# diver-j/melgan-multi

Hardware: NVIDIA H100
Metric: generator_fwd_audio_frames_per_sec (higher is better)
Workload: dtype f32 in/out; products as 3 split-bf16 wgmma passes with fp32 accumulation (fp32-equivalent, ~1e-5)

## Files before the change

### include/melgan_b200.h

```cpp
#ifndef MELGAN_B200_H_
#define MELGAN_B200_H_

#include <stddef.h>
#include <stdint.h>

#ifdef __cplusplus
extern "C" {
#endif

#define MG_OK 0
#define MG_ERR_INVALID_ARGUMENT (-1)
#define MG_ERR_CUDA (-2)
#define MG_ERR_UNSUPPORTED_DEVICE (-3)
#define MG_ERR_WORKSPACE_TOO_SMALL (-4)
#define MG_ERR_OUT_OF_MEMORY (-5)

#define MG_GEN_NUM_LAYERS 30

int mg_abi_version(void);

const char *mg_last_error_string(void);

int mg_device_check(void);

size_t mg_gen_packed_bytes(void);
int mg_gen_pack(const float *const *v, const float *const *g, const float *const *bias,
                void *packed, void *stream);

size_t mg_gen_workspace_bytes(int B, int T);
int mg_gen_forward(const void *packed, const float *mel, float *audio, int B, int T,
                   void *workspace, size_t workspace_bytes, void *stream);

#define MG_GEN_RAGGED_MAX_B 256
int mg_gen_forward_ragged(const void *packed, const float *mel, float *audio, int B, int T_max, const int *lengths,
                          void *workspace, size_t workspace_bytes, void *stream);

int mg_gen_forward_timed(const void *packed, const float *mel, float *audio, int B, int T,
                         void *workspace, size_t workspace_bytes, void *stream, float *kernel_ms);

int mg_gen_check_status(const void *workspace, int B, int T, void *stream);

int mg_gen_convt(const void *packed, int stage, const float *x, float *y, int B, int Lin, void *stream);

int mg_gen_resblock(const void *packed, int stage, const float *x, float *y, int B, int L, void *stream);
int mg_gen_upres(const void *packed, int stage, const float *x, float *y, int B, int Lin, void *stream);
int mg_gen_upres_post(const void *packed, const float *x, float *audio, int B, int Lin, void *stream);
const char *mg_gen_resblock_config(int code);
const char *mg_gen_convt_config(int stage);

int mg_gen_resup(const void *packed, int stage, const float *x, float *y, int B, int L, void *stream);

int mg_gen_conv_pre(const void *packed, const float *mel, float *y, int B, int T, void *stream);
int mg_gen_resblock_post(const void *packed, const float *x, float *audio, int B, int L, void *stream);

int mg_gen_resblock_trace(const void *packed, int stage, const float *x, float *y, int B, int L, long long *trace_host);

int mg_gen_stage_output(const void *workspace, int which, float *out, int B, int T, void *stream);

size_t mg_msd_packed_bytes(void);
int mg_msd_pack(const float *const *v, const float *const *g, const float *const *bias, void *packed, void *stream);
int mg_msd_lengths(int L, int *lens);
int mg_msd_forward(const void *packed, const float *y, int Bt, int L, float *const *fmaps, void *status_word, void *stream);
int mg_msd_check_status(const void *status_word, void *stream);

size_t mg_disc_packed_bytes(void);
int mg_disc_pack(const float *const *v, const float *const *g, const float *const *bias, void *packed, void *stream);
int mg_disc_forward(const void *packed, const float *x, int Bt, int L, float *const *fmaps, void *status_word, void *stream);

size_t mg_mel_tables_bytes(void);
int mg_mel_tables_build(int sampling_rate, int n_mels, float fmin, float fmax, int norm, void *tables_host);
int mg_mel_frames(int L);
int mg_mel_spectrogram(const void *tables, const float *audio, float *mel, int B, int L, void *stream);

typedef struct mg_gen_engine mg_gen_engine;

int mg_gen_engine_create(mg_gen_engine **out, int max_B, int max_T);
int mg_gen_engine_load_state(mg_gen_engine *e, const float *const *v, const float *const *g,
                             const float *const *bias);
int mg_gen_engine_forward(mg_gen_engine *e, const float *mel_host, float *audio_host, int B, int T);
int mg_gen_engine_forward_ragged(mg_gen_engine *e, const float *mel_host, float *audio_host, int B, int T_max,
                                 const int *lengths);
int mg_gen_engine_last_kernel_ms(mg_gen_engine *e, float *ms);
void mg_gen_engine_destroy(mg_gen_engine *e);


size_t mg_msd_scale_backward_workspace_bytes(int Bt, int L0);
int mg_msd_scale_backward(const void *packed, int scale, const float *x0, const float *const *fmap, const float *const *gfmap,
                          float *gx0, float *const *dw, float *const *db, int *reached, void *workspace, size_t workspace_bytes,
                          int Bt, int L0, void *status_word, void *stream);

int mg_lrelu_backward(const float *g1, const float *g2, const float *out, float *dz, long long n, void *stream);

size_t mg_msd_grouped_backward_workspace_bytes(int layer, int Bt, int Lout);
int mg_msd_grouped_backward(const void *packed, int scale, int layer, const float *dz, const float *x, float *dx, float *dw,
                            float *db, void *workspace, size_t workspace_bytes, int Bt, int Lin, int Lout, void *stream);

int mg_msd_post1_dgrad(const void *packed, int scale, const float *dz, float *dx, int Bt, int L, void *status_word, void *stream);
int mg_msd_post1_wgrad(const float *x, const float *dz, float *dw, float *db, int Bt, int L, void *status_word, void *stream);

size_t mg_msd_edge_backward_workspace_bytes(int layer, int Bt, int L);
int mg_msd_edge_backward(const void *packed, int scale, int layer, const float *dz, const float *x, float *dx, float *dw, float *db,
                         void *workspace, size_t workspace_bytes, int Bt, int L, void *stream);

int mg_msd_wn_backward(const float *const *v, const float *const *g, const float *const *dw, float *const *dv,
                       float *const *dg, void *stream);

int mg_adam_chunk(void);
int mg_adam_step(float *const *p, const float *const *g, float *const *m, float *const *v, const long long *n,
                 const int *first, int count, int total_ctas, float lr, float beta1, float beta2, float eps,
                 float weight_decay, long long step, void *stream);

size_t mg_loss_workspace_bytes(const long long *n, int count);
int mg_loss_forward(const float *const *a, const float *const *b, const long long *n, const int *mode, int count,
                    float *out, void *workspace, size_t workspace_bytes, void *stream);
int mg_loss_backward(const float *const *a, const float *const *b, const long long *n, const int *mode, int count,
                     const float *grad_out, float *const *grad_a, float *const *grad_b, void *stream);

int mg_gen_forward_launches(void);
int mg_gen_forward_slices(int B, int T);
int mg_gen_set_pipeline(int tail_mask);
const char *mg_gen_kernel_name(int i);
const char *mg_gen_kernel_config(int i, int T);

#ifdef __cplusplus
}
#endif
#endif
```

### melgan_multi_b200/csrc/mg_api.cu

```cuda
#include <new>
#include <stdlib.h>
#include <string.h>

#include "mg_common.cuh"

namespace mg {


static int *status_ptr(void *workspace, int B, int T) {
    return reinterpret_cast<int *>(reinterpret_cast<float *>(workspace) + ws_offset(6, (size_t)B, (size_t)T));
}

static int run_generator(const float *packed, const float *mel, float *audio, const RunTable &batch, float *ws, cudaStream_t s,
                         cudaEvent_t *ev, const float *mel_host = nullptr, float *audio_host = nullptr) {
    int *st = status_ptr(ws, batch.items(), batch.stride);
    MG_CUDA_TRY(cudaMemsetAsync(st, 0, sizeof(int), s));
    return launch_generator_tc(packed, mel, audio, batch, ws, st, s, ev, mel_host, audio_host);
}

static int check_shape(const char *fn, int B, int T) {
    if (B < 1 || T < 1) return set_error(MG_ERR_INVALID_ARGUMENT, "%s: need B >= 1 and T >= 1 (got B=%d, T=%d)", fn, B, T);
    if ((long long)B * T > (1ll << 24)) return set_error(MG_ERR_INVALID_ARGUMENT, "%s: B*T = %lld too large", fn, (long long)B * T);
    return MG_OK;
}

static int check_lengths(const char *fn, int B, int T_max, const int *lengths) {
    int rc = check_shape(fn, B, T_max);
    if (rc) return rc;
    if (B > MG_GEN_RAGGED_MAX_B)
        return set_error(MG_ERR_INVALID_ARGUMENT, "%s: B = %d exceeds MG_GEN_RAGGED_MAX_B = %d", fn, B, MG_GEN_RAGGED_MAX_B);
    if (!lengths) return set_error(MG_ERR_INVALID_ARGUMENT, "%s: null lengths", fn);
    for (int i = 0; i < B; ++i)
        if (lengths[i] < 1 || lengths[i] > T_max)
            return set_error(MG_ERR_INVALID_ARGUMENT, "%s: lengths[%d] = %d is outside [1, T_max = %d]", fn, i, lengths[i], T_max);
    return MG_OK;
}

template <class F>
static int run_one_kernel(const char *fn, cudaStream_t stream, F launch) {
    int *st = nullptr;
    MG_CUDA_TRY(cudaMalloc(&st, sizeof(int)));
    cudaMemsetAsync(st, 0, sizeof(int), stream);
    int rc = launch(st);
    int h = 0;
    if (rc == MG_OK) {
        cudaError_t e = cudaStreamSynchronize(stream);
        if (e != cudaSuccess) rc = set_error(MG_ERR_CUDA, "%s: %s", fn, cudaGetErrorString(e));
        else if (cudaMemcpy(&h, st, sizeof(int), cudaMemcpyDeviceToHost) != cudaSuccess || h)
            rc = set_error(MG_ERR_CUDA, "%s: pipeline wait timed out (role code %d)", fn, h);
    }
    cudaFree(st);
    return rc;
}

}

using namespace mg;

extern "C" {

int mg_abi_version(void) { return 2; }

const char *mg_last_error_string(void) { return error_buffer(); }

int mg_device_check(void) {
    int dev = 0;
    MG_CUDA_TRY(cudaGetDevice(&dev));
    cudaDeviceProp p;
    MG_CUDA_TRY(cudaGetDeviceProperties(&p, dev));
    if (p.major != 9 || p.minor != 0)
        return set_error(MG_ERR_UNSUPPORTED_DEVICE, "device %d is sm_%d%d; this library is built for sm_90a (H100) only",
                         dev, p.major, p.minor);
    return MG_OK;
}

size_t mg_gen_packed_bytes(void) { return packed_total_bytes(); }

int mg_gen_pack(const float *const *v, const float *const *g, const float *const *bias, void *packed, void *stream) {
    if (!v || !g || !bias || !packed) return set_error(MG_ERR_INVALID_ARGUMENT, "mg_gen_pack: null argument");
    if ((uintptr_t)packed % 16) return set_error(MG_ERR_INVALID_ARGUMENT, "mg_gen_pack: packed must be 16-byte aligned");
    return launch_pack(v, g, bias, (float *)packed, (cudaStream_t)stream);
}

size_t mg_gen_workspace_bytes(int B, int T) {
    if (B < 1 || T < 1) return 0;
    return ws_offset(6, (size_t)B, (size_t)T) * sizeof(float) + 256;
}

static int check_forward(const char *fn, const void *packed, const float *mel, float *audio, int B, int T, void *workspace,
                         size_t workspace_bytes) {
    if (!packed || !mel || !audio || !workspace) return set_error(MG_ERR_INVALID_ARGUMENT, "%s: null argument", fn);
    if (workspace_bytes < mg_gen_workspace_bytes(B, T))
        return set_error(MG_ERR_WORKSPACE_TOO_SMALL, "%s: workspace %zu < %zu bytes", fn, workspace_bytes, mg_gen_workspace_bytes(B, T));
    if ((uintptr_t)packed % 16 || (uintptr_t)workspace % 16)
        return set_error(MG_ERR_INVALID_ARGUMENT, "%s: packed/workspace must be 16-byte aligned", fn);
    return MG_OK;
}

int mg_gen_forward(const void *packed, const float *mel, float *audio, int B, int T, void *workspace,
                   size_t workspace_bytes, void *stream) {
    int rc = check_shape("mg_gen_forward", B, T);
    if (!rc) rc = check_forward("mg_gen_forward", packed, mel, audio, B, T, workspace, workspace_bytes);
    if (rc) return rc;
    return run_generator((const float *)packed, mel, audio, RunTable::uniform(B, T), (float *)workspace, (cudaStream_t)stream,
                         nullptr);
}

int mg_gen_forward_ragged(const void *packed, const float *mel, float *audio, int B, int T_max, const int *lengths,
                          void *workspace, size_t workspace_bytes, void *stream) {
    int rc = check_lengths("mg_gen_forward_ragged", B, T_max, lengths);
    if (!rc) rc = check_forward("mg_gen_forward_ragged", packed, mel, audio, B, T_max, workspace, workspace_bytes);
    if (rc) return rc;
    return run_generator((const float *)packed, mel, audio, RunTable::ragged(lengths, B, T_max), (float *)workspace,
                         (cudaStream_t)stream, nullptr);
}

int mg_gen_forward_timed(const void *packed, const float *mel, float *audio, int B, int T, void *workspace,
                         size_t workspace_bytes, void *stream, float *kernel_ms) {
    int rc = check_shape("mg_gen_forward_timed", B, T);
    if (rc) return rc;
    if (!packed || !mel || !audio || !workspace || !kernel_ms)
        return set_error(MG_ERR_INVALID_ARGUMENT, "mg_gen_forward_timed: null argument");
    if (workspace_bytes < mg_gen_workspace_bytes(B, T))
        return set_error(MG_ERR_WORKSPACE_TOO_SMALL, "mg_gen_forward_timed: workspace too small");
    const int n = mg_gen_forward_launches();
    cudaEvent_t ev[17];
    for (int i = 0; i <= n; ++i) MG_CUDA_TRY(cudaEventCreate(&ev[i]));
    rc = run_generator((const float *)packed, mel, audio, RunTable::uniform(B, T), (float *)workspace, (cudaStream_t)stream, ev);
    if (rc == MG_OK) {
        cudaError_t e = cudaEventSynchronize(ev[n]);
        if (e != cudaSuccess) rc = set_error(MG_ERR_CUDA, "mg_gen_forward_timed: %s", cudaGetErrorString(e));
        for (int i = 0; i < n && rc == MG_OK; ++i)
            if (cudaEventElapsedTime(&kernel_ms[i], ev[i], ev[i + 1]) != cudaSuccess)
                rc = set_error(MG_ERR_CUDA, "mg_gen_forward_timed: cudaEventElapsedTime failed");
    }
    for (int i = 0; i <= n; ++i) cudaEventDestroy(ev[i]);
    return rc;
}

const char *mg_gen_kernel_name(int i) { return generator_tc_kernel_name(i); }

const char *mg_gen_kernel_config(int i, int T) { return generator_tc_kernel_config(i, T); }

int mg_gen_set_pipeline(int tail_mask) {
    if (tail_mask < -1 || tail_mask > 15) return set_error(MG_ERR_INVALID_ARGUMENT, "mg_gen_set_pipeline: mask %d", tail_mask);
    generator_tc_set_tail(tail_mask);
    return MG_OK;
}

int mg_gen_stage_output(const void *workspace, int which, float *out, int B, int T, void *stream) {
    int rc = check_shape("mg_gen_stage_output", B, T);
    if (rc) return rc;
    if (which < 0 || which > 3 || !workspace || !out)
        return set_error(MG_ERR_INVALID_ARGUMENT, "mg_gen_stage_output: which must be 0..3 (the last stage is fused with conv_post)");
    if (which > 0 && generator_tc_tail() != 0)
        return set_error(MG_ERR_INVALID_ARGUMENT, "mg_gen_stage_output: ResBlock outputs are not materialised while the next stage's "
                         "ConvT is fused at their kernel's tail; select the unfused chain with mg_gen_set_pipeline(0) first");
    const size_t off = ws_offset(which, B, T), n = ws_offset(which + 1, B, T) - off;
    MG_CUDA_TRY(cudaMemcpyAsync(out, (const float *)workspace + off, n * sizeof(float), cudaMemcpyDeviceToDevice,
                                (cudaStream_t)stream));
    return MG_OK;
}

size_t mg_msd_grouped_backward_workspace_bytes(int layer, int Bt, int Lout) {
    if (layer < 1 || layer > 4 || Bt < 1 || Lout < 1) return 0;
    return grouped_bwd_workspace_bytes(layer, Bt, Lout);
}

int mg_msd_grouped_backward(const void *packed, int scale, int layer, const float *dz, const float *x, float *dx, float *dw,
                            float *db, void *workspace, size_t workspace_bytes, int Bt, int Lin, int Lout, void *stream) {
    if (!packed || !dz || scale < 0 || scale > 2 || layer < 1 || layer > 4 || Bt < 1 || Lin < 1 || Lout < 1)
        return set_error(MG_ERR_INVALID_ARGUMENT, "mg_msd_grouped_backward: bad argument");
    const DLayer d = d_layer(layer);
    if (Lout != (Lin + 2 * d.pad - d.k) / d.stride + 1)
        return set_error(MG_ERR_INVALID_ARGUMENT, "mg_msd_grouped_backward: Lout %d does not follow from Lin %d", Lout, Lin);
    if (dw && (!x || !db || !workspace || workspace_bytes < grouped_bwd_workspace_bytes(layer, Bt, Lout)))
        return set_error(MG_ERR_WORKSPACE_TOO_SMALL, "mg_msd_grouped_backward: dw needs x, db and a workspace of %zu bytes",
                         grouped_bwd_workspace_bytes(layer, Bt, Lout));
    const uint8_t *blob = reinterpret_cast<const uint8_t *>(packed) + (size_t)scale * d_blob_bytes();
    return launch_disc_grouped_backward(blob, layer, dz, x, dx, dw, db, (float *)workspace, Bt, Lin, Lout, (cudaStream_t)stream);
}

int mg_msd_post1_dgrad(const void *packed, int scale, const float *dz, float *dx, int Bt, int L, void *status_word, void *stream) {
    if (!packed || !dz || !dx || dz == dx || !status_word || scale < 0 || scale > 2 || Bt < 1 || L < 1)
        return set_error(MG_ERR_INVALID_ARGUMENT, "mg_msd_post1_dgrad: bad argument");
    const uint8_t *blob = reinterpret_cast<const uint8_t *>(packed) + (size_t)scale * d_blob_bytes();
    return launch_disc_post1_dgrad_tc(dz, dx, blob + d_tcT_start(), reinterpret_cast<const float *>(blob + d_zero_start()), Bt, L,
                                      (int *)status_word, (cudaStream_t)stream);
}

int mg_msd_post1_wgrad(const float *x, const float *dz, float *dw, float *db, int Bt, int L, void *status_word, void *stream) {
    if (!x || !dz || !dw || !db || !status_word || Bt < 1 || L < 1)
        return set_error(MG_ERR_INVALID_ARGUMENT, "mg_msd_post1_wgrad: bad argument");
    return launch_disc_post1_wgrad_tc(x, dz, dw, db, Bt, L, (int *)status_word, (cudaStream_t)stream);
}

size_t mg_msd_edge_backward_workspace_bytes(int layer, int Bt, int L) {
    return (layer == 0 && Bt > 0 && L > 0) ? edge_bwd_workspace_bytes(layer, Bt, L) : 0;
}

int mg_msd_edge_backward(const void *packed, int scale, int layer, const float *dz, const float *x, float *dx, float *dw, float *db,
                         void *workspace, size_t workspace_bytes, int Bt, int L, void *stream) {
    if (!packed || !dz || !x || !dw || !db || scale < 0 || scale > 2 || (layer != 0 && layer != 6) || Bt < 1 || L < 1)
        return set_error(MG_ERR_INVALID_ARGUMENT, "mg_msd_edge_backward: bad argument (layer is 0 = conv_pre or 6 = conv_post2)");
    if (layer == 0 && (!workspace || workspace_bytes < edge_bwd_workspace_bytes(0, Bt, L)))
        return set_error(MG_ERR_WORKSPACE_TOO_SMALL, "mg_msd_edge_backward: conv_pre needs a workspace of %zu bytes",
                         edge_bwd_workspace_bytes(0, Bt, L));
    const uint8_t *blob = reinterpret_cast<const uint8_t *>(packed) + (size_t)scale * d_blob_bytes();
    return launch_disc_edge_backward(blob, layer, dz, x, dx, dw, db, (float *)workspace, Bt, L, (cudaStream_t)stream);
}

size_t mg_msd_scale_backward_workspace_bytes(int Bt, int L0) {
    return (Bt > 0 && L0 > 0) ? disc_scale_backward_workspace_bytes(Bt, L0) : 0;
}

int mg_msd_scale_backward(const void *packed, int scale, const float *x0, const float *const *fmap, const float *const *gfmap,
                          float *gx0, float *const *dw, float *const *db, int *reached, void *workspace, size_t workspace_bytes,
                          int Bt, int L0, void *status_word, void *stream) {
    if (!packed || !x0 || !fmap || !gfmap || !dw || !db || !workspace || !status_word || scale < 0 || scale > 2 || Bt < 1 || L0 < 1)
        return set_error(MG_ERR_INVALID_ARGUMENT, "mg_msd_scale_backward: bad argument");
    for (int l = 0; l < kDiscLayers; ++l)
        if (!fmap[l]) return set_error(MG_ERR_INVALID_ARGUMENT, "mg_msd_scale_backward: fmap[%d] is NULL", l);
    if (Bt > 65535) return set_error(MG_ERR_INVALID_ARGUMENT, "discriminator batch %d exceeds 65535", Bt);
    const uint8_t *blob = reinterpret_cast<const uint8_t *>(packed) + (size_t)scale * d_blob_bytes();
    return launch_disc_scale_backward(blob, x0, fmap, gfmap, gx0, dw, db, reached, workspace, workspace_bytes, Bt, L0,
                                      (int *)status_word, (cudaStream_t)stream);
}

int mg_lrelu_backward(const float *g1, const float *g2, const float *out, float *dz, long long n, void *stream) {
    return launch_lrelu_grad(g1, g2, out, dz, n, (cudaStream_t)stream);
}

int mg_msd_wn_backward(const float *const *v, const float *const *g, const float *const *dw, float *const *dv,
                       float *const *dg, void *stream) {
    if (!v || !g || !dw || !dv || !dg) return set_error(MG_ERR_INVALID_ARGUMENT, "mg_msd_wn_backward: null argument");
    return launch_disc_wn_backward(v, g, dw, dv, dg, (cudaStream_t)stream);
}

int mg_adam_chunk(void) { return 4096; }

int mg_adam_step(float *const *p, const float *const *g, float *const *m, float *const *v, const long long *n,
                 const int *first, int count, int total_ctas, float lr, float beta1, float beta2, float eps,
                 float weight_decay, long long step, void *stream) {
    return launch_adam(p, g, m, v, n, first, count, total_ctas, lr, beta1, beta2, eps, weight_decay, step, (cudaStream_t)stream);
}

size_t mg_loss_workspace_bytes(const long long *n, int count) {
    if (!n || count < 1) return 0;
    return (size_t)loss_num_ctas(n, count) * sizeof(float);
}

int mg_loss_forward(const float *const *a, const float *const *b, const long long *n, const int *mode, int count,
                    float *out, void *workspace, size_t workspace_bytes, void *stream) {
    if (!out || !workspace) return set_error(MG_ERR_INVALID_ARGUMENT, "mg_loss_forward: null argument");
    if (n && count >= 1 && workspace_bytes < mg_loss_workspace_bytes(n, count))
        return set_error(MG_ERR_WORKSPACE_TOO_SMALL, "mg_loss_forward: workspace too small");
    return launch_loss_forward(a, b, n, mode, count, out, (float *)workspace, (cudaStream_t)stream);
}

int mg_loss_backward(const float *const *a, const float *const *b, const long long *n, const int *mode, int count,
                     const float *grad_out, float *const *grad_a, float *const *grad_b, void *stream) {
    if (!grad_out) return set_error(MG_ERR_INVALID_ARGUMENT, "mg_loss_backward: null grad_out");
    return launch_loss_backward(a, b, n, mode, count, grad_out, grad_a, grad_b, (cudaStream_t)stream);
}

int mg_gen_forward_launches(void) { return generator_tc_num_launches(); }

int mg_gen_forward_slices(int B, int T) { return (B >= 1 && T >= 1) ? generator_tc_slices(B, (long long)B * T) : 1; }

int mg_gen_check_status(const void *workspace, int B, int T, void *stream) {
    int rc = check_shape("mg_gen_check_status", B, T);
    if (rc) return rc;
    if (!workspace) return set_error(MG_ERR_INVALID_ARGUMENT, "mg_gen_check_status: null workspace");
    MG_CUDA_TRY(cudaStreamSynchronize((cudaStream_t)stream));
    int st = 0;
    MG_CUDA_TRY(cudaMemcpy(&st, status_ptr(const_cast<void *>(workspace), B, T), sizeof(int), cudaMemcpyDeviceToHost));
    if (st) return set_error(MG_ERR_CUDA, "tensor-core pipeline wait timed out (role code %d)", st);
    return MG_OK;
}

int mg_gen_convt(const void *packed, int stage, const float *x, float *y, int B, int Lin, void *stream) {
    if (!packed || !x || !y || x == y || stage < 0 || stage > 3 || B < 1 || Lin < 1)
        return set_error(MG_ERR_INVALID_ARGUMENT, "mg_gen_convt: bad argument");
    return run_one_kernel("mg_gen_convt", (cudaStream_t)stream, [&](int *st) {
        return launch_convt_tc(x, y, (const float *)packed, stage, RunTable::uniform(B, Lin), st, (cudaStream_t)stream);
    });
}

int mg_gen_conv_pre(const void *packed, const float *mel, float *y, int B, int T, void *stream) {
    if (!packed || !mel || !y || B < 1 || T < 1) return set_error(MG_ERR_INVALID_ARGUMENT, "mg_gen_conv_pre: bad argument");
    return run_one_kernel("mg_gen_conv_pre", (cudaStream_t)stream, [&](int *st) {
        return launch_gen_pre_tc(mel, y, (const float *)packed, RunTable::uniform(B, T), st, (cudaStream_t)stream);
    });
}

int mg_gen_resblock_post(const void *packed, const float *x, float *audio, int B, int L, void *stream) {
    if (!packed || !x || !audio || B < 1 || L < 1) return set_error(MG_ERR_INVALID_ARGUMENT, "mg_gen_resblock_post: bad argument");
    return run_one_kernel("mg_gen_resblock_post", (cudaStream_t)stream, [&](int *st) {
        return launch_resblock_tc(x, audio, (const float *)packed, 4, RunTable::uniform(B, L), st, (cudaStream_t)stream);
    });
}

int mg_gen_resblock_trace(const void *packed, int stage, const float *x, float *y, int B, int L, long long *trace_host) {
    if (!packed || !x || !y || x == y || !trace_host || !*resblock_config_name(stage, 0) || B < 1 || L < 1)
        return set_error(MG_ERR_INVALID_ARGUMENT, "mg_gen_resblock_trace: bad argument");
    int *st = nullptr;
    long long *tr = nullptr;
    MG_CUDA_TRY(cudaMalloc(&st, sizeof(int)));
    MG_CUDA_TRY(cudaMalloc(&tr, 128 * sizeof(long long)));
    cudaMemset(st, 0, sizeof(int));
    cudaMemset(tr, 0, 128 * sizeof(long long));
    int rc = launch_resblock_tc(x, y, (const float *)packed, stage, RunTable::uniform(B, L), st, 0, tr);
    if (rc == MG_OK && cudaDeviceSynchronize() != cudaSuccess) rc = set_error(MG_ERR_CUDA, "mg_gen_resblock_trace: kernel failed");
    if (rc == MG_OK) cudaMemcpy(trace_host, tr, 128 * sizeof(long long), cudaMemcpyDeviceToHost);
    cudaFree(st);
    cudaFree(tr);
    return rc;
}

int mg_gen_resblock(const void *packed, int stage, const float *x, float *y, int B, int L, void *stream) {
    if (!packed || !x || !y || x == y || stage < 0 || stage > 3 || B < 1 || L < 1)
        return set_error(MG_ERR_INVALID_ARGUMENT, "mg_gen_resblock: bad argument");
    return run_one_kernel("mg_gen_resblock", (cudaStream_t)stream, [&](int *st) {
        return launch_resblock_tc(x, y, (const float *)packed, stage, RunTable::uniform(B, L), st, (cudaStream_t)stream);
    });
}

int mg_gen_resup(const void *packed, int stage, const float *x, float *y, int B, int L, void *stream) {
    if (!packed || !x || !y || x == y || stage < 0 || stage > 2 || B < 1 || L < 1)
        return set_error(MG_ERR_INVALID_ARGUMENT, "mg_gen_resup: bad argument");
    return run_one_kernel("mg_gen_resup", (cudaStream_t)stream, [&](int *st) {
        return launch_resblock_tc(x, y, (const float *)packed, 20 + stage, RunTable::uniform(B, L), st, (cudaStream_t)stream);
    });
}

int mg_gen_upres(const void *packed, int stage, const float *x, float *y, int B, int Lin, void *stream) {
    if (!packed || !x || !y || x == y || (stage != 2 && stage != 3) || B < 1 || Lin < 1)
        return set_error(MG_ERR_INVALID_ARGUMENT, "mg_gen_upres: bad argument");
    return run_one_kernel("mg_gen_upres", (cudaStream_t)stream, [&](int *st) {
        return launch_resblock_tc(x, y, (const float *)packed, 10 + stage, RunTable::uniform(B, 2 * Lin), st, (cudaStream_t)stream);
    });
}

int mg_gen_upres_post(const void *packed, const float *x, float *audio, int B, int Lin, void *stream) {
    if (!packed || !x || !audio || (const void *)x == (const void *)audio || B < 1 || Lin < 1)
        return set_error(MG_ERR_INVALID_ARGUMENT, "mg_gen_upres_post: bad argument");
    return run_one_kernel("mg_gen_upres_post", (cudaStream_t)stream, [&](int *st) {
        return launch_resblock_tc(x, audio, (const float *)packed, 14, RunTable::uniform(B, 2 * Lin), st, (cudaStream_t)stream);
    });
}

const char *mg_gen_resblock_config(int code) { return resblock_config_name(code, 0); }
const char *mg_gen_convt_config(int stage) { return convt_config_name(stage); }


size_t mg_msd_packed_bytes(void) { return msd_packed_bytes(); }

int mg_msd_pack(const float *const *v, const float *const *g, const float *const *bias, void *packed, void *stream) {
    if (!v || !g || !bias || !packed) return set_error(MG_ERR_INVALID_ARGUMENT, "mg_msd_pack: null argument");
    if ((uintptr_t)packed % 256) return set_error(MG_ERR_INVALID_ARGUMENT, "mg_msd_pack: packed must be 256-byte aligned");
    return launch_disc_pack(v, g, bias, packed, (cudaStream_t)stream);
}

int mg_msd_lengths(int L, int *lens) {
    if (L < 1 || !lens) return set_error(MG_ERR_INVALID_ARGUMENT, "mg_msd_lengths: bad argument");
    msd_lengths(L, lens);
    for (int i = 0; i < 21; ++i)
        if (lens[i] < 1) return set_error(MG_ERR_INVALID_ARGUMENT, "mg_msd_lengths: L = %d is too short for the discriminators", L);
    return MG_OK;
}

int mg_msd_forward(const void *packed, const float *y, int Bt, int L, float *const *fmaps, void *status_word, void *stream) {
    if (!packed || !y || !fmaps || !status_word || Bt < 1 || L < 1)
        return set_error(MG_ERR_INVALID_ARGUMENT, "mg_msd_forward: bad argument");
    int lens[21];
    int rc = mg_msd_lengths(L, lens);
    if (rc) return rc;
    for (int i = 0; i < 21; ++i)
        if (!fmaps[i]) return set_error(MG_ERR_INVALID_ARGUMENT, "mg_msd_forward: null feature-map pointer %d", i);
    MG_CUDA_TRY(cudaMemsetAsync(status_word, 0, sizeof(int), (cudaStream_t)stream));
    return launch_msd_forward(packed, y, Bt, L, fmaps, (int *)status_word, (cudaStream_t)stream);
}

size_t mg_disc_packed_bytes(void) { return d_blob_bytes(); }

int mg_disc_pack(const float *const *v, const float *const *g, const float *const *bias, void *packed, void *stream) {
    if (!v || !g || !bias || !packed) return set_error(MG_ERR_INVALID_ARGUMENT, "mg_disc_pack: null argument");
    if ((uintptr_t)packed % 256) return set_error(MG_ERR_INVALID_ARGUMENT, "mg_disc_pack: packed must be 256-byte aligned");
    return launch_disc_pack(v, g, bias, packed, (cudaStream_t)stream, 1);
}

int mg_disc_forward(const void *packed, const float *x, int Bt, int L, float *const *fmaps, void *status_word, void *stream) {
    if (!packed || !x || !fmaps || !status_word || Bt < 1 || L < 1)
        return set_error(MG_ERR_INVALID_ARGUMENT, "mg_disc_forward: bad argument");
    int lens[21];
    msd_lengths(L, lens);
    for (int i = 0; i < 7; ++i) {
        if (lens[i] < 1) return set_error(MG_ERR_INVALID_ARGUMENT, "mg_disc_forward: L = %d is too short", L);
        if (!fmaps[i]) return set_error(MG_ERR_INVALID_ARGUMENT, "mg_disc_forward: null feature-map pointer %d", i);
    }
    MG_CUDA_TRY(cudaMemsetAsync(status_word, 0, sizeof(int), (cudaStream_t)stream));
    return launch_disc_forward(packed, x, Bt, L, fmaps, (int *)status_word, (cudaStream_t)stream);
}

int mg_msd_check_status(const void *status_word, void *stream) {
    if (!status_word) return set_error(MG_ERR_INVALID_ARGUMENT, "mg_msd_check_status: null argument");
    MG_CUDA_TRY(cudaStreamSynchronize((cudaStream_t)stream));
    int st = 0;
    MG_CUDA_TRY(cudaMemcpy(&st, status_word, sizeof(int), cudaMemcpyDeviceToHost));
    if (st) return set_error(MG_ERR_CUDA, "tensor-core pipeline wait timed out (role code %d)", st);
    return MG_OK;
}


size_t mg_mel_tables_bytes(void) { return mel_tables_bytes(); }

int mg_mel_tables_build(int sampling_rate, int n_mels, float fmin, float fmax, int norm, void *tables_host) {
    if (!tables_host) return set_error(MG_ERR_INVALID_ARGUMENT, "mg_mel_tables_build: null buffer");
    return mel_tables_build(sampling_rate, n_mels, fmin, fmax, norm, reinterpret_cast<MelTables *>(tables_host));
}

int mg_mel_frames(int L) { return L < 1 ? 0 : mel_frames(L); }

int mg_mel_spectrogram(const void *tables, const float *audio, float *mel, int B, int L, void *stream) {
    if (!tables || !audio || !mel || B < 1 || L < 1) return set_error(MG_ERR_INVALID_ARGUMENT, "mg_mel_spectrogram: bad argument");
    if ((uintptr_t)tables % 16) return set_error(MG_ERR_INVALID_ARGUMENT, "mg_mel_spectrogram: tables must be 16-byte aligned");
    return launch_mel(tables, audio, mel, B, L, (cudaStream_t)stream);
}


struct mg_gen_engine {
    cudaStream_t stream = nullptr;
    cudaEvent_t ev0 = nullptr, ev1 = nullptr;
    float *packed = nullptr;
    float *raw = nullptr;
    float *mel = nullptr, *audio = nullptr, *ws = nullptr;
    float *pin_in = nullptr, *pin_out = nullptr;
    int *pin_status = nullptr;
    size_t cap_frames = 0;
    bool loaded = false;
    float last_ms = 0.f;
};

static void engine_free_io(mg_gen_engine *e) {
    cudaFree(e->mel); cudaFree(e->audio); cudaFree(e->ws);
    cudaFreeHost(e->pin_in); cudaFreeHost(e->pin_out);
    e->mel = e->audio = e->ws = e->pin_in = e->pin_out = nullptr;
    e->cap_frames = 0;
}

static int engine_reserve(mg_gen_engine *e, size_t frames) {
    if (frames <= e->cap_frames) return MG_OK;
    engine_free_io(e);
    MG_CUDA_TRY(cudaMalloc(&e->mel, frames * kMelBins * sizeof(float)));
    MG_CUDA_TRY(cudaMalloc(&e->audio, frames * 256 * sizeof(float)));
    MG_CUDA_TRY(cudaMalloc(&e->ws, mg_gen_workspace_bytes(1, (int)frames)));
    MG_CUDA_TRY(cudaMallocHost(&e->pin_in, frames * kMelBins * sizeof(float)));
    MG_CUDA_TRY(cudaMallocHost(&e->pin_out, frames * 256 * sizeof(float)));
    e->cap_frames = frames;
    return MG_OK;
}

int mg_gen_engine_create(mg_gen_engine **out, int max_B, int max_T) {
    if (!out) return set_error(MG_ERR_INVALID_ARGUMENT, "mg_gen_engine_create: null out");
    int rc = check_shape("mg_gen_engine_create", max_B, max_T);
    if (rc) return rc;
    if ((rc = mg_device_check())) return rc;
    mg_gen_engine *e = new (std::nothrow) mg_gen_engine();
    if (!e) return set_error(MG_ERR_OUT_OF_MEMORY, "mg_gen_engine_create: host allocation failed");
    *out = e;
    MG_CUDA_TRY(cudaStreamCreateWithFlags(&e->stream, cudaStreamNonBlocking));
    MG_CUDA_TRY(cudaEventCreate(&e->ev0));
    MG_CUDA_TRY(cudaEventCreate(&e->ev1));
    MG_CUDA_TRY(cudaMalloc((void **)&e->packed, mg_gen_packed_bytes()));
    MG_CUDA_TRY(cudaMalloc(&e->raw, (packed_float_count() + 4353) * sizeof(float)));
    return engine_reserve(e, (size_t)max_B * max_T);
}

int mg_gen_engine_load_state(mg_gen_engine *e, const float *const *v, const float *const *g, const float *const *bias) {
    if (!e || !v || !g || !bias) return set_error(MG_ERR_INVALID_ARGUMENT, "mg_gen_engine_load_state: null argument");
    const float *dv[kNumLayers], *dg[kNumLayers], *db[kNumLayers];
    float *p = e->raw;
    for (int l = 0; l < kNumLayers; ++l) {
        if (!v[l] || !g[l] || !bias[l]) return set_error(MG_ERR_INVALID_ARGUMENT, "mg_gen_engine_load_state: null tensor, layer %d", l);
        const size_t nv = layer_weight_count(l), ng = layer_norm_rows(l), nb = layer_shape(l).cout;
        MG_CUDA_TRY(cudaMemcpyAsync(p, v[l], nv * sizeof(float), cudaMemcpyHostToDevice, e->stream)); dv[l] = p; p += nv;
        MG_CUDA_TRY(cudaMemcpyAsync(p, g[l], ng * sizeof(float), cudaMemcpyHostToDevice, e->stream)); dg[l] = p; p += ng;
        MG_CUDA_TRY(cudaMemcpyAsync(p, bias[l], nb * sizeof(float), cudaMemcpyHostToDevice, e->stream)); db[l] = p; p += nb;
    }
    int rc = launch_pack(dv, dg, db, e->packed, e->stream);
    if (rc) return rc;
    MG_CUDA_TRY(cudaStreamSynchronize(e->stream));
    e->loaded = true;
    return MG_OK;
}

static int engine_check(const char *fn, mg_gen_engine *e, const float *mel_host, float *audio_host) {
    if (!e || !mel_host || !audio_host) return set_error(MG_ERR_INVALID_ARGUMENT, "%s: null argument", fn);
    if (!e->loaded) return set_error(MG_ERR_INVALID_ARGUMENT, "%s: no weights loaded", fn);
    return MG_OK;
}

static int engine_forward(mg_gen_engine *e, const float *mel_host, float *audio_host, const RunTable &batch) {
    const int B = batch.items(), T = batch.stride;
    const size_t frames = (size_t)B * T;
    int rc = engine_reserve(e, frames);
    if (rc) return rc;
    const size_t nin = frames * kMelBins * sizeof(float), nout = frames * 256 * sizeof(float);
    cudaPointerAttributes at;
    const bool in_pinned = cudaPointerGetAttributes(&at, mel_host) == cudaSuccess && at.type == cudaMemoryTypeHost;
    const bool out_pinned = cudaPointerGetAttributes(&at, audio_host) == cudaSuccess && at.type == cudaMemoryTypeHost;
    cudaGetLastError();
    const float *src = mel_host;
    if (!in_pinned) { memcpy(e->pin_in, mel_host, nin); src = e->pin_in; }
    if (!e->pin_status) MG_CUDA_TRY(cudaMallocHost(&e->pin_status, sizeof(int)));
    MG_CUDA_TRY(cudaEventRecord(e->ev0, e->stream));
    rc = run_generator(e->packed, e->mel, e->audio, batch, e->ws, e->stream, nullptr, src, out_pinned ? audio_host : e->pin_out);
    if (rc) return rc;
    MG_CUDA_TRY(cudaEventRecord(e->ev1, e->stream));
    *e->pin_status = 0;
    MG_CUDA_TRY(cudaMemcpyAsync(e->pin_status, status_ptr(e->ws, B, T), sizeof(int), cudaMemcpyDeviceToHost, e->stream));
    MG_CUDA_TRY(cudaStreamSynchronize(e->stream));
    if (!out_pinned) memcpy(audio_host, e->pin_out, nout);
    if (*e->pin_status)
        return set_error(MG_ERR_CUDA, "mg_gen_engine_forward: tensor-core pipeline wait timed out (code %d)", *e->pin_status);
    MG_CUDA_TRY(cudaEventElapsedTime(&e->last_ms, e->ev0, e->ev1));
    return MG_OK;
}

int mg_gen_engine_forward(mg_gen_engine *e, const float *mel_host, float *audio_host, int B, int T) {
    int rc = engine_check("mg_gen_engine_forward", e, mel_host, audio_host);
    if (!rc) rc = check_shape("mg_gen_engine_forward", B, T);
    return rc ? rc : engine_forward(e, mel_host, audio_host, RunTable::uniform(B, T));
}

int mg_gen_engine_forward_ragged(mg_gen_engine *e, const float *mel_host, float *audio_host, int B, int T_max, const int *lengths) {
    int rc = check_lengths("mg_gen_engine_forward_ragged", B, T_max, lengths);
    if (!rc) rc = engine_check("mg_gen_engine_forward_ragged", e, mel_host, audio_host);
    return rc ? rc : engine_forward(e, mel_host, audio_host, RunTable::ragged(lengths, B, T_max));
}

int mg_gen_engine_last_kernel_ms(mg_gen_engine *e, float *ms) {
    if (!e || !ms) return set_error(MG_ERR_INVALID_ARGUMENT, "mg_gen_engine_last_kernel_ms: null argument");
    *ms = e->last_ms;
    return MG_OK;
}

void mg_gen_engine_destroy(mg_gen_engine *e) {
    if (!e) return;
    engine_free_io(e);
    cudaFree(e->packed); cudaFree(e->raw);
    if (e->pin_status) cudaFreeHost(e->pin_status);
    if (e->ev0) cudaEventDestroy(e->ev0);
    if (e->ev1) cudaEventDestroy(e->ev1);
    if (e->stream) cudaStreamDestroy(e->stream);
    delete e;
}

}
```

### melgan_multi_b200/csrc/mg_common.cuh

```cuda
#pragma once
#include <cuda_runtime.h>
#include <stdarg.h>
#include <stdint.h>
#include <stdio.h>

#include "../../include/melgan_b200.h"
#include "mg_layout.h"

namespace mg {

constexpr int kNumSMs = 132;

char *error_buffer();
int set_error(int code, const char *fmt, ...);

#define MG_CUDA_TRY(expr)                                                                     \
    do {                                                                                      \
        cudaError_t err__ = (expr);                                                           \
        if (err__ != cudaSuccess)                                                             \
            return ::mg::set_error(MG_ERR_CUDA, "%s failed: %s (%s:%d)", #expr,               \
                                   cudaGetErrorString(err__), __FILE__, __LINE__);            \
    } while (0)

__device__ __forceinline__ float lrelu(float x) { return fmaxf(x, x * kSlope); }

__device__ __forceinline__ void cp_async16(void *smem_dst, const void *gmem_src) {
    uint32_t d = (uint32_t)__cvta_generic_to_shared(smem_dst);
    asm volatile("cp.async.cg.shared.global [%0], [%1], 16;\n" ::"r"(d), "l"(gmem_src));
}
__device__ __forceinline__ void cp_async_commit() { asm volatile("cp.async.commit_group;\n" ::); }
template <int N>
__device__ __forceinline__ void cp_async_wait() {
    asm volatile("cp.async.wait_group %0;\n" ::"n"(N));
}

struct RunPos {
    int item, unit, len;
};
struct RunTable {
    int n, stride;
    int item0[MG_GEN_RAGGED_MAX_B + 1], len[MG_GEN_RAGGED_MAX_B];
    int first[MG_GEN_RAGGED_MAX_B + 1], per[MG_GEN_RAGGED_MAX_B];

    static RunTable uniform(int B, int L) {
        RunTable t;
        t.n = 1;
        t.stride = L;
        t.item0[0] = 0;
        t.item0[1] = B;
        t.len[0] = L;
        return t;
    }
    static RunTable ragged(const int *lengths, int B, int stride) {
        RunTable t;
        t.n = 0;
        t.stride = stride;
        for (int i = 0; i < B; ++i)
            if (i == 0 || lengths[i] != lengths[i - 1]) {
                t.item0[t.n] = i;
                t.len[t.n++] = lengths[i];
            }
        t.item0[t.n] = B;
        return t;
    }
    int items() const { return item0[n]; }
    RunTable slice(int i0, int i1) const {
        RunTable t;
        t.n = 0;
        t.stride = stride;
        for (int r = 0; r < n; ++r) {
            const int a = item0[r] > i0 ? item0[r] : i0, b = item0[r + 1] < i1 ? item0[r + 1] : i1;
            if (a < b) {
                t.item0[t.n] = a - i0;
                t.len[t.n++] = len[r];
            }
        }
        t.item0[t.n] = i1 - i0;
        return t;
    }
    RunTable scaled(int k) const {
        RunTable t = *this;
        t.stride *= k;
        for (int r = 0; r < n; ++r) t.len[r] *= k;
        return t;
    }
    template <class F>
    void set_units(F units) {
        first[0] = 0;
        for (int r = 0; r < n; ++r) {
            per[r] = units(len[r]);
            first[r + 1] = first[r] + (item0[r + 1] - item0[r]) * per[r];
        }
    }
    __device__ __forceinline__ RunPos find(int f) const {
        if (f < 0 || f >= first[n]) return {-1, 0, 0};
        int lo = 0, hi = n;
        while (hi - lo > 1) {
            const int m = (lo + hi) >> 1;
            if (first[m] <= f) lo = m;
            else hi = m;
        }
        const int u = f - first[lo], k = (int)((unsigned)u / (unsigned)per[lo]);
        return {item0[lo] + k, u - k * per[lo], len[lo]};
    }
};

bool pdl_enabled();
template <class... KArgs, class... Args>
inline cudaError_t launch_ex(void (*kernel)(KArgs...), dim3 grid, dim3 block, size_t smem, cudaStream_t s, bool pdl, int cluster,
                             Args... args) {
    cudaLaunchConfig_t cfg{};
    cfg.gridDim = grid;
    cfg.blockDim = block;
    cfg.dynamicSmemBytes = smem;
    cfg.stream = s;
    cudaLaunchAttribute attr[2];
    int n = 0;
    if (pdl && pdl_enabled()) {
        attr[n].id = cudaLaunchAttributeProgrammaticStreamSerialization;
        attr[n].val.programmaticStreamSerializationAllowed = 1;
        ++n;
    }
    if (cluster > 1) {
        attr[n].id = cudaLaunchAttributeClusterDimension;
        attr[n].val.clusterDim.x = cluster;
        attr[n].val.clusterDim.y = 1;
        attr[n].val.clusterDim.z = 1;
        ++n;
    }
    cfg.attrs = attr;
    cfg.numAttrs = n;
    return cudaLaunchKernelEx(&cfg, kernel, static_cast<KArgs>(args)...);
}

int launch_pack(const float *const *v, const float *const *g, const float *const *bias, float *packed,
                cudaStream_t s);
int launch_generator_simt(const float *packed, const float *mel, float *audio, int B, int T, float *ws,
                          cudaStream_t s, cudaEvent_t *ev = nullptr);
int generator_simt_num_launches();
int generator_tc_num_launches();
int generator_tc_fused_up();
int generator_tc_tail();
void generator_tc_set_tail(int mask);
const char *generator_tc_kernel_name(int i);
const char *generator_tc_kernel_config(int i, int T);
const char *resblock_config_name(int stage, int L);
int generator_tc_slices(int B, long long frames);
int launch_generator_tc(const float *packed, const float *mel, float *audio, const RunTable &batch, float *ws, int *status,
                        cudaStream_t s, cudaEvent_t *ev = nullptr, const float *mel_host = nullptr, float *audio_host = nullptr);
int launch_gen_pre_tc(const float *mel, float *y, const float *packed, const RunTable &batch, int *status, cudaStream_t s);
int launch_disc_post1_tc(const float *x, float *y, const uint8_t *wtc, const float *bias, int Bt, int L, int *status,
                         cudaStream_t s);
int launch_disc_post1_dgrad_tc(const float *dz, float *dx, const uint8_t *wtcT, const float *zero_bias, int Bt, int L, int *status,
                               cudaStream_t s);
int launch_disc_post1_wgrad_tc(const float *x, const float *dz, float *dw, float *db, int Bt, int L, int *status, cudaStream_t s);
size_t disc_scale_backward_workspace_bytes(int Bt, int L0);
int launch_disc_scale_backward(const void *blob, const float *x0, const float *const *fmap, const float *const *gfmap, float *gx0,
                               float *const *dw, float *const *db, int *reached, void *workspace, size_t workspace_bytes, int Bt,
                               int L0, int *status, cudaStream_t st);
size_t edge_bwd_workspace_bytes(int l, int Bt, int L);
int launch_disc_edge_backward(const void *blob, int l, const float *dz, const float *x, float *dx, float *dw, float *db, float *ws,
                              int Bt, int L, cudaStream_t s);
int launch_disc_group_tc(const float *x, float *out, const uint8_t *wtc, const float *bias, int Bt, int Cin, int Cout,
                         int Lin, int Lout, int *status, cudaStream_t s);
int launch_disc_group4_tc(const float *x, float *out, const uint8_t *wtc, const float *bias, int Bt, int L, int *status,
                          cudaStream_t s);
int launch_disc_pack(const float *const *v, const float *const *g, const float *const *bias, void *packed, cudaStream_t s, int ndisc = 3);
int launch_disc_forward(const void *packed, const float *x, int Bt, int L, float *const *fmaps, int *status, cudaStream_t s);
void msd_lengths(int L, int *lens);
int launch_lrelu_grad(const float *g1, const float *g2, const float *out, float *dz, long long n, cudaStream_t s);
size_t grouped_bwd_workspace_bytes(int l, int Bt, int Lout);
int launch_disc_grouped_backward(const void *blob, int l, const float *dz, const float *x, float *dx, float *dw, float *db,
                                 float *ws, int Bt, int Lin, int Lout, cudaStream_t s);
int launch_disc_wn_backward(const float *const *v, const float *const *g, const float *const *dw, float *const *dv,
                            float *const *dg, cudaStream_t s);
int launch_adam(float *const *p, const float *const *g, float *const *m, float *const *v, const long long *n, const int *first,
                int count, int total_ctas, float lr, float b1, float b2, float eps, float wd, long long step, cudaStream_t s);
long long loss_num_ctas(const long long *n, int count);
int launch_loss_forward(const float *const *a, const float *const *b, const long long *n, const int *mode, int count, float *out,
                        float *partial, cudaStream_t s);
int launch_loss_backward(const float *const *a, const float *const *b, const long long *n, const int *mode, int count,
                         const float *gout, float *const *ga, float *const *gb, cudaStream_t s);
struct MelTables;
size_t mel_tables_bytes();
int mel_tables_build(int sr, int n_mels, float fmin, float fmax, int norm, MelTables *t);
int mel_frames(int L);
int launch_mel(const void *tables, const float *audio, float *mel, int B, int L, cudaStream_t s);
int launch_msd_forward(const void *packed, const float *y, int Bt, int L, float *const *fmaps, int *status, cudaStream_t s);
int launch_convt_tc(const float *x, float *y, const float *packed, int stage, const RunTable &batch, int *status, cudaStream_t s);
const char *convt_config_name(int stage);
int launch_resblock_tc(const float *x, float *y, const float *packed, int stage, const RunTable &batch, int *status, cudaStream_t s,
                       long long *trace = nullptr);

}
```

### melgan_multi_b200/csrc/mg_res_tc.cu

```cuda
#include <stdlib.h>
#include <string.h>

#include "mg_common.cuh"
#include "mg_tc.cuh"

namespace mg {
using namespace tc;

template <int C_, int NRB_, int RPW_, int NCP_, int NSTAGE_, bool POST_ = false, bool UPF_ = false, int UPT_ = 0, int CS_ = 1>
struct RbCfg {
    static constexpr int C = C_, NRB = NRB_, RPW = RPW_, NCP = NCP_, NSTAGE = NSTAGE_, UPT = UPT_, CS = CS_;
    static constexpr bool POST = POST_;
    static constexpr bool UPF = UPF_;
    static constexpr int P = 64 * NRB;
    static constexpr int NWG = NRB / RPW * NCP;
    static constexpr int NCONS = 128 * NWG;
    static constexpr int NT = NCONS + 32;
    static constexpr int NCW = C / NCP;
    static constexpr int SLACK = 16;
    static constexpr int HALO = 16 + (POST ? 3 : 0);
    static constexpr int HL = HALO + (UPT_ ? 1 : 0);
    static constexpr int ROWS = P + 2 * SLACK;
    static constexpr int XPITCH = ROWS * 16;
    static constexpr int KP = C / 8;
    static constexpr int XBYTES = KP * XPITCH;
    static constexpr int KC = tc_kc(C);
    static constexpr int CHUNK = tc_chunk_bytes(C);
    static constexpr int HALF = CHUNK / 2;
    static constexpr int NCHUNK = tc_chunks_per_conv(C);
    static constexpr int KSL = C / KC;
    static constexpr int TNG = UPT == 8 ? 32 : C / 2, TN = (UPT ? UPT : 1) * TNG, TNCG = (C / 2) / TNG;
    static constexpr int TSLOT = UPT == 8 ? 16384 : 128 * UPT * TNG, TNSLOT = UPT ? TNCG * (C / 16) * (UPT == 8 ? 2 : 1) : 0;
    static_assert(UPT == 0 || ((UPT == 2 || UPT == 8) && TN == C && TSLOT <= CHUNK && !POST_ && !UPF_), "tail ConvT shape");
    static_assert(UPT != 8 || NCW == 128, "stride-8 tail: each column part stores four phases of a channel as one float4");
    static constexpr int UROWS = P / 2 + 2, UPITCH = UROWS * 16, NPB = NRB / 2, UKSL = 2 * C / KC, NUPCH = UPF ? 4 * UKSL : 0;
    static constexpr int SPITCH = P + 4;
    static_assert(!UPF || (NCP == 1 && NPB <= NWG && 2 * KP * UPITCH <= XBYTES && C * SPITCH * 4 <= 2 * XBYTES),
                  "fused ConvT must fit the X region");
    static_assert(!POST || (C == 32 && NCP == 1), "conv_post fusion is for the 32-channel stage");
    static constexpr int PVB = CS * P - HALO - HL, XCH = 9;
    static_assert(CS == 1 || ((CS == 2 || CS == 4) && !POST_ && !UPF_ && UPT_ == 0 && XCH <= SLACK && 2 * XCH <= P),
                  "clusters are for the plain ResBlock");
    static constexpr int CB_UPF = 6 * C, CB_UPT = CB_UPF + (UPF_ ? C : 0), CB_POST = CB_UPT + (UPT_ ? C / 2 : 0);
    static constexpr int NCONST = CB_POST + (POST_ ? 32 * 8 + 4 : 0);
    static_assert(CB_POST % 4 == 0 && NCONST % 2 == 0, "conv_post weights are read as float4, the mbarriers follow");
    static constexpr int SMEM_BYTES = 2 * XBYTES + NSTAGE * CHUNK + (2 * C + NCONST) * 4 + (2 * NSTAGE + (CS > 1 ? 2 : 0) + 1) * 8;
    static_assert(SMEM_BYTES + 1024 <= 227 * 1024, "shared memory budget");
    static_assert(XPITCH / 16 < 16384, "LBO field");
    static_assert(NRB % RPW == 0 && C % NCP == 0 && NCW % 32 == 0, "warpgroup split");
};

template <int RPW, int R>
__device__ __forceinline__ void acc_fence2(float (&a)[RPW][R]) {
#pragma unroll
    for (int r = 0; r < RPW; ++r) acc_fence<R>(a[r]);
}

template <class Cfg>
__global__ void __launch_bounds__(Cfg::NT, 1)
resblock_tc_kernel(const float *__restrict__ x, float *__restrict__ y, const float *__restrict__ packed, int stage,
                   const __grid_constant__ RunTable clusters, int *__restrict__ status, long long *__restrict__ trace) {
    constexpr int C = Cfg::C, P = Cfg::P, SLACK = Cfg::SLACK, HALO = Cfg::HALO, HL = Cfg::HL;
    constexpr int XPITCH = Cfg::XPITCH, XBYTES = Cfg::XBYTES, KC = Cfg::KC, CHUNK = Cfg::CHUNK, NSTAGE = Cfg::NSTAGE;
    constexpr int NCONS = Cfg::NCONS, NCP = Cfg::NCP, NCW = Cfg::NCW, RPW = Cfg::RPW, KSL = Cfg::KSL, NA = NCW / 2;
    constexpr int CS = Cfg::CS, XCH = Cfg::XCH;
    extern __shared__ __align__(1024) uint8_t smem[];
    uint8_t *Xh = smem, *Xl = smem + XBYTES, *ring = smem + 2 * XBYTES;
    float *pend = reinterpret_cast<float *>(ring + NSTAGE * CHUNK);
    float *b1s = pend + C;
    float *cst = b1s + C;
    uint64_t *full = reinterpret_cast<uint64_t *>(cst + Cfg::NCONST);
    uint64_t *empty = full + NSTAGE;
    uint64_t *hfull = empty + NSTAGE, *hfree = hfull + 1;
    int *item_len = reinterpret_cast<int *>(empty + NSTAGE + (CS > 1 ? 2 : 0));

    const int tid = threadIdx.x, warp = tid >> 5, lane = tid & 31;
    const int crank = blockIdx.x % CS;
    const RunPos cp = clusters.find(blockIdx.x / CS);
    const int clus = cp.unit, Ls = clusters.stride;
    auto item = [&]() { return *reinterpret_cast<volatile int *>(&item_len[0]); };
    auto len = [&]() { return *reinterpret_cast<volatile int *>(&item_len[1]); };
    const int oc = clus == 0 ? 0 : (CS * P - HALO) + (clus - 1) * Cfg::PVB - HL;
    const int o = oc + crank * P;
    const int p_lo = (clus == 0 || crank > 0) ? 0 : HL, p_hi = (crank < CS - 1 || oc + CS * P >= cp.len) ? P : P - HALO;
    const bool interior = (o >= 0 && o + P <= cp.len);
    const int l0 = 5 + 6 * stage;
    const uint8_t *tc_base = reinterpret_cast<const uint8_t *>(packed) + tc_region_start();

    if (tid == 0) {
        item_len[0] = cp.item;
        item_len[1] = cp.len;
        for (int s = 0; s < NSTAGE; ++s) {
            mbar_init(&full[s], 1);
            mbar_init(&empty[s], Cfg::NWG * CS);
        }
        if constexpr (CS > 1) {
            mbar_init(hfull, 1);
            mbar_init(hfree, (crank > 0) + (crank < CS - 1));
        }
        fence_mbar_init();
    }
    for (int i = Cfg::UPF ? 1 << 30 : tid; i < 2 * Cfg::KP * 2 * SLACK; i += Cfg::NT) {
        const int r = i % (2 * SLACK), kp = (i / (2 * SLACK)) % Cfg::KP, hl = i / (2 * SLACK * Cfg::KP);
        const int row = r < SLACK ? r : P + r;
        *reinterpret_cast<uint4 *>((hl ? Xl : Xh) + kp * XPITCH + row * 16) = make_uint4(0, 0, 0, 0);
    }
    for (int i = tid; i < C; i += Cfg::NT) pend[i] = 0.f;
    for (int i = tid; i < Cfg::NCONST; i += Cfg::NT) {
        float v = 0.f;
        if (i < Cfg::CB_UPF) v = __ldg(packed + bias_offset(l0) + i);
        else if (i < Cfg::CB_UPT) v = __ldg(packed + bias_offset(1 + stage) + (i - Cfg::CB_UPF));
        else if (i < Cfg::CB_POST) v = __ldg(packed + bias_offset(1 + stage + 1) + (i - Cfg::CB_UPT));
        else if (i < Cfg::CB_POST + 32 * 8) {
            const int j = i - Cfg::CB_POST;
            if ((j & 7) < kPostK) v = __ldg(packed + weight_offset(29) + (j >> 3) * kPostK + (j & 7));
        } else if (i == Cfg::CB_POST + 32 * 8) {
            v = __ldg(packed + bias_offset(29));
        }
        cst[i] = v;
    }
    fence_proxy_async();
    __syncthreads();
    if constexpr (CS > 1) cluster_sync();
    const bool tr = trace && blockIdx.x == (gridDim.x > 1 ? 1u : 0u) && tid == 0;
#define MG_TR(slot) do { if (tr) trace[slot] = clock64(); } while (0)

    if (warp == NCONS / 32) {
        if (lane == 0) {
            int s = 0, ph = 0, j = 0;
            bool ok = true;
            auto put = [&](const uint8_t *src, uint32_t bytes) {
                if (!ok || !mbar_wait(&empty[s], ph ^ 1)) { ok = false; return; }
                mbar_arrive_expect_tx(&full[s], bytes);
                if constexpr (CS == 1) bulk_g2s(ring + s * CHUNK, src, bytes, &full[s]);
                else if (j % CS == crank) bulk_g2s_multicast(ring + s * CHUNK, src, bytes, &full[s], (1 << CS) - 1);
                ++j;
                if (++s == NSTAGE) { s = 0; ph ^= 1; }
            };
            if constexpr (Cfg::UPF) {
                const uint8_t *src = tc_base + tc_upf_offset(stage);
                for (int i = 0; i < Cfg::NUPCH; ++i) put(src + (size_t)i * CHUNK, CHUNK);
            }
            for (int conv = 0; conv < 6; ++conv) {
                const uint8_t *src = tc_base + tc_res_offset(l0 + (conv >> 1) + 3 * (conv & 1));
                for (int i = 0; i < Cfg::NCHUNK; ++i) put(src + (size_t)i * CHUNK, CHUNK);
            }
            if constexpr (Cfg::UPT != 0) {
                const uint8_t *src = tc_base + tc_up_offset(stage + 1);
                for (int i = 0; i < Cfg::TNSLOT; ++i) put(src + (size_t)i * Cfg::TSLOT, Cfg::TSLOT);
            }
            if (!ok) atomicExch(status, 2);
        }
        if constexpr (CS > 1) cluster_sync();
        return;
    }

    const int wgi = warp >> 2, t = tid & 127, q = lane & 3;
    const int rb0 = (wgi / NCP) * RPW, c0 = (wgi % NCP) * NCW;
    const uint64_t adesc_t = desc_template(XPITCH, 128), bdesc_t = desc_template(C * 16, 128);
    const uint32_t xh_addr = smem_u32(Xh), xl_addr = smem_u32(Xl), ring_addr = smem_u32(ring);
    float R[RPW][NA], D[RPW][NA];
    int s = 0, ph = 0, ps = -1;
    bool ok = true;
    auto release = [&](int slot) {
        if constexpr (CS == 1) {
            if (t == 0) mbar_arrive(&empty[slot]);
        } else if (t < CS) {
            mbar_arrive_remote(&empty[slot], t);
        }
    };
    auto chunk_begin = [&]() -> uint32_t {
        ok &= mbar_wait(&full[s], ph);
        acc_fence2(R);
        acc_fence2(D);
        wgmma_fence();
        return ring_addr + s * CHUNK;
    };
    auto chunk_end = [&]() {
        wgmma_commit();
        wgmma_wait<1>();
        if (ps >= 0) release(ps);
        ps = s;
        if (++s == NSTAGE) { s = 0; ph ^= 1; }
    };
    auto drain = [&]() {
        wgmma_wait<0>();
        acc_fence2(R);
        acc_fence2(D);
        if (ps >= 0) release(ps);
        ps = -1;
    };
    auto sync_cons = [&]() { named_bar_sync(1, NCONS); };
    const int nbr = tid == 0 ? crank - 1 : crank + 1;
    const bool tells = tid < 2 && nbr >= 0 && nbr < CS;
    auto x_read = [&]() {
        sync_cons();
        if constexpr (CS > 1)
            if (tells) mbar_arrive_remote(hfree, nbr);
    };
    auto write_x = [&](float (&A)[RPW][NA], const float *bsrc, bool keep_last) {
        const int L = len();
#pragma unroll
        for (int r = 0; r < RPW; ++r)
#pragma unroll
            for (int h = 0; h < 2; ++h) {
                const int p = (rb0 + r) * 64 + frag_row(t, h), tp = o + p;
                const bool inr = interior || (tp >= 0 && tp < L);
                uint8_t *xh = Xh + (c0 >> 3) * XPITCH + (p + SLACK) * 16 + q * 4, *xl = xh + XBYTES;
#pragma unroll
                for (int k = 0; k < NCW / 8; ++k) {
                    const int col = c0 + 8 * k + 2 * q;
                    const float2 bb = *reinterpret_cast<const float2 *>(bsrc + col);
                    const float f0 = inr ? lrelu(A[r][4 * k + 2 * h] + bb.x) : 0.f;
                    const float f1 = inr ? lrelu(A[r][4 * k + 2 * h + 1] + bb.y) : 0.f;
                    uint32_t hi, lo;
                    split2_bf16(f0, f1, hi, lo);
                    *reinterpret_cast<uint32_t *>(xh + k * XPITCH) = hi;
                    *reinterpret_cast<uint32_t *>(xl + k * XPITCH) = lo;
                    if (keep_last && tp == L - 1) *reinterpret_cast<float2 *>(b1s + col) = make_float2(f0, f1);
                }
            }
    };
    bool border = false;
#pragma unroll
    for (int r = 0; r < RPW; ++r)
#pragma unroll
        for (int h = 0; h < 2; ++h) {
            const int p = (rb0 + r) * 64 + frag_row(t, h);
            border |= (crank > 0 && p < XCH) || (crank < CS - 1 && p >= P - XCH);
        }
    constexpr int NXC = 2 * Cfg::KP;
    constexpr uint32_t XCB = XCH * 16;
    constexpr int NW = NCONS / 32;
    auto send_halo = [&]() {
        for (int i = warp + NW * lane; i < 2 * NXC; i += NCONS) {
            const int side = i / NXC, nb = side ? crank + 1 : crank - 1;
            if (nb < 0 || nb >= CS) continue;
            const uint32_t panel = xh_addr + (i % NXC) * XPITCH;
            const int src = side ? P - XCH : 0, dst = side ? -XCH : P;
            bulk_s2s_cluster(mapa(panel + (SLACK + dst) * 16, nb), panel + (SLACK + src) * 16, XCB, mapa(smem_u32(hfull), nb));
        }
    };
    int hand = 0;
    auto hand_off = [&](float (&A)[RPW][NA], const float *bsrc, bool keep_last) {
        if constexpr (CS > 1) {
            if (border && hand > 0) {
                MG_TR(100 + 2 * hand);
                ok &= mbar_wait(hfree, (hand - 1) & 1);
                MG_TR(101 + 2 * hand);
            }
            if (tid == 0) mbar_arrive_expect_tx(hfull, ((crank > 0) + (crank < CS - 1)) * NXC * XCB);
        }
        write_x(A, bsrc, keep_last);
        fence_proxy_async();
        sync_cons();
        if constexpr (CS > 1) send_halo();
        ++hand;
    };
    auto conv_mma = [&](float (&A)[RPW][NA], int dil, bool fresh, int conv) {
        if constexpr (CS > 1) {
            MG_TR(88 + 2 * conv);
            ok &= mbar_wait(hfull, conv & 1);
            MG_TR(89 + 2 * conv);
        }
        MG_TR(64 + 3 * conv);
#pragma unroll 1
        for (int ch = 0; ch < Cfg::NCHUNK; ++ch) {
            const int tap = ch / KSL, ks = ch % KSL;
            const uint64_t bbase = desc_at(bdesc_t, chunk_begin() + c0 * 16);
            if (ch == 0) MG_TR(65 + 3 * conv);
            const uint32_t arow = (SLACK + rb0 * 64 + (tap - 1) * dil) * 16 + ks * (KC / 8) * XPITCH;
#pragma unroll
            for (int pass = 0; pass < 3; ++pass)
#pragma unroll
                for (int k16 = 0; k16 < KC / 16; ++k16) {
                    const uint64_t bdesc = bbase + (uint64_t)(((pass == 2 ? Cfg::HALF : 0) + 2 * k16 * (C * 16)) >> 4);
                    const uint64_t adesc = desc_at(adesc_t, (pass == 1 ? xl_addr : xh_addr) + arow + 2 * k16 * XPITCH);
#pragma unroll
                    for (int r = 0; r < RPW; ++r)
                        wgmma_bf16<NCW>(A[r], adesc + (uint64_t)(r * 64), bdesc, !(fresh && ch == 0 && pass == 0 && k16 == 0));
                }
            chunk_end();
        }
        MG_TR(66 + 3 * conv);
        drain();
    };

    pdl_wait();
    MG_TR(0);
    if constexpr (Cfg::UPF) {
        constexpr int UROWS = Cfg::UROWS, UPITCH = Cfg::UPITCH, SPITCH = Cfg::SPITCH, UKSL = Cfg::UKSL;
        const int b = item(), L = len();
        const int Lin = L >> 1, Lins = Ls >> 1, s0 = (o >> 1) - 1;
#pragma unroll 1
        for (int idx = tid; idx < UROWS * 2 * Cfg::KP; idx += NCONS) {
            const int i = idx % UROWS, kp = idx / UROWS, sp = s0 + i;
            const bool inr = (sp >= 0 && sp < Lin);
            const float *xp = x + ((size_t)b * 2 * C + 8 * kp) * Lins + (inr ? sp : 0);
            float f[8];
#pragma unroll
            for (int j = 0; j < 8; ++j) f[j] = inr ? lrelu(__ldg(xp + (size_t)j * Lins)) : 0.f;
            uint32_t h[4], l[4];
#pragma unroll
            for (int e = 0; e < 4; ++e) split2_bf16(f[2 * e], f[2 * e + 1], h[e], l[e]);
            *reinterpret_cast<uint4 *>(Xh + kp * UPITCH + i * 16) = make_uint4(h[0], h[1], h[2], h[3]);
            *reinterpret_cast<uint4 *>(Xl + kp * UPITCH + i * 16) = make_uint4(l[0], l[1], l[2], l[3]);
        }
        fence_proxy_async();
        sync_cons();
        const uint64_t udesc_t = desc_template(UPITCH, 128);
        const bool mine = wgi < Cfg::NPB;
        const int pb = wgi % Cfg::NPB;
        auto upf_tap = [&](float (&A)[RPW][NA], int k) {
            const int rowoff = (k == 0) ? 2 : (k == 3) ? 0 : 1;
#pragma unroll 1
            for (int ks = 0; ks < UKSL; ++ks) {
                const uint64_t bbase = desc_at(bdesc_t, chunk_begin());
                const uint32_t arow = (rowoff + pb * 64) * 16 + ks * (KC / 8) * UPITCH;
#pragma unroll
                for (int pass = 0; pass < 3; ++pass)
#pragma unroll
                    for (int k16 = 0; k16 < KC / 16; ++k16) {
                        const uint64_t bdesc = bbase + (uint64_t)(((pass == 2 ? Cfg::HALF : 0) + 2 * k16 * (C * 16)) >> 4);
                        const uint64_t adesc = desc_at(udesc_t, (pass == 1 ? xl_addr : xh_addr) + arow + 2 * k16 * UPITCH);
                        wgmma_bf16<NCW>(A[0], adesc, bdesc, !(k < 2 && ks == 0 && pass == 0 && k16 == 0));
                    }
                chunk_end();
            }
        };
        upf_tap(D, 0);
        upf_tap(R, 1);
        upf_tap(D, 2);
        upf_tap(R, 3);
        drain();
        sync_cons();
        float *stg = reinterpret_cast<float *>(Xh);
        const float *ubias = cst + Cfg::CB_UPF;
        if (mine) {
#pragma unroll
            for (int h = 0; h < 2; ++h) {
                const int m = wgi * 64 + frag_row(t, h);
#pragma unroll
                for (int j = 0; j < NA; ++j) {
                    const int col = frag_col(q, (j & ~3) | (j & 1));
                    if ((j & 2) == 2 * h) {
                        const float bj = ubias[col];
                        *reinterpret_cast<float2 *>(stg + (size_t)col * SPITCH + 2 * m) = make_float2(R[0][j] + bj, D[0][j] + bj);
                    }
                }
            }
        }
        sync_cons();
#pragma unroll
        for (int r = 0; r < RPW; ++r)
#pragma unroll
            for (int j = 0; j < NA; ++j) {
                const int p = (rb0 + r) * 64 + frag_row(t, (j >> 1) & 1);
                R[r][j] = stg[(size_t)frag_col(q, (j & ~3) | (j & 1)) * SPITCH + p];
            }
        sync_cons();
        for (int i = tid; i < 2 * Cfg::KP * 2 * SLACK; i += NCONS) {
            const int r = i % (2 * SLACK), kp = (i / (2 * SLACK)) % Cfg::KP, hl = i / (2 * SLACK * Cfg::KP);
            const int row = r < SLACK ? r : P + r;
            *reinterpret_cast<uint4 *>((hl ? Xl : Xh) + kp * XPITCH + row * 16) = make_uint4(0, 0, 0, 0);
        }
    } else {
        const int b = item(), L = len();
#pragma unroll
        for (int r = 0; r < RPW; ++r)
#pragma unroll
            for (int h = 0; h < 2; ++h) {
                const int p = (rb0 + r) * 64 + frag_row(t, h), tp = o + p;
                const bool inr = (tp >= 0 && tp < L);
                const float *xp = x + (size_t)b * C * Ls + (inr ? tp : 0);
#pragma unroll
                for (int k = 0; k < NCW / 8; ++k)
#pragma unroll
                    for (int e = 0; e < 2; ++e)
                        R[r][4 * k + 2 * h + e] = inr ? __ldg(xp + (size_t)(c0 + frag_col(q, 4 * k + e)) * Ls) : 0.f;
            }
    }
    hand_off(R, pend, false);
    MG_TR(1);

#pragma unroll 1
    for (int pr = 0; pr < 3; ++pr) {
        MG_TR(2 + 6 * pr);
        conv_mma(D, pr == 0 ? 1 : pr == 1 ? 3 : 9, true, 2 * pr);
        MG_TR(3 + 6 * pr);
        x_read();
        hand_off(D, cst + pr * C, false);
        MG_TR(4 + 6 * pr);
        for (int c = tid; c < C; c += NCONS) pend[c] += cst[(3 + pr) * C + c];
        MG_TR(5 + 6 * pr);
        conv_mma(R, 1, false, 2 * pr + 1);
        MG_TR(6 + 6 * pr);
        x_read();
        if (pr < 2 || Cfg::UPT != 0) hand_off(R, pend, Cfg::UPT != 0 && pr == 2);
        MG_TR(7 + 6 * pr);
    }

    if constexpr (Cfg::POST) {
        pdl_trigger();
        float *Q = reinterpret_cast<float *>(Xh);
        const float *wpost = cst + Cfg::CB_POST;
#pragma unroll
        for (int r = 0; r < RPW; ++r)
#pragma unroll
            for (int h = 0; h < 2; ++h) {
                const int p = (rb0 + r) * 64 + frag_row(t, h), tp = o + p;
                const bool inr = (tp >= 0 && tp < len());
                float qk[kPostK];
#pragma unroll
                for (int k = 0; k < kPostK; ++k) qk[k] = 0.f;
#pragma unroll
                for (int k = 0; k < NCW / 8; ++k)
#pragma unroll
                    for (int e = 0; e < 2; ++e) {
                        const int ci = frag_col(q, 4 * k + e);
                        const float a = inr ? lrelu(R[r][4 * k + 2 * h + e] + pend[ci]) : 0.f;
                        const float4 w0 = *reinterpret_cast<const float4 *>(wpost + ci * 8);
                        const float4 w1 = *reinterpret_cast<const float4 *>(wpost + ci * 8 + 4);
                        qk[0] = fmaf(w0.x, a, qk[0]); qk[1] = fmaf(w0.y, a, qk[1]); qk[2] = fmaf(w0.z, a, qk[2]);
                        qk[3] = fmaf(w0.w, a, qk[3]); qk[4] = fmaf(w1.x, a, qk[4]); qk[5] = fmaf(w1.y, a, qk[5]);
                        qk[6] = fmaf(w1.z, a, qk[6]);
                    }
#pragma unroll
                for (int k = 0; k < kPostK; ++k) {
                    qk[k] += __shfl_xor_sync(0xffffffffu, qk[k], 1);
                    qk[k] += __shfl_xor_sync(0xffffffffu, qk[k], 2);
                }
                if (q == 0) {
#pragma unroll
                    for (int k = 0; k < kPostK; ++k) Q[k * P + p] = qk[k];
                }
            }
        sync_cons();
        const int b = item(), L = len();
        const float bpost = cst[Cfg::CB_POST + 32 * 8];
#pragma unroll 1
        for (int p = tid; p < P; p += NCONS) {
            const int tp = o + p;
            if (p >= p_lo && p < p_hi && tp < L) {
                float acc = bpost;
#pragma unroll
                for (int k = 0; k < kPostK; ++k) {
                    const int pp = p + k - 3;
                    if (pp >= 0 && pp < P) acc += Q[k * P + pp];
                }
                y[(size_t)b * Ls + tp] = tanhf(acc);
            }
        }
        if (oc + P >= L)
            for (int p = L + tid; p < Ls; p += NCONS) y[(size_t)b * Ls + p] = 0.f;
    } else if constexpr (Cfg::UPT != 0) {
        constexpr int S = Cfg::UPT, TNG = Cfg::TNG, TN = Cfg::TN, PADT = S / 2, COT = C / 2;
        const int b = item(), L = len();
        const int Lout = S * Ls;
        const float *tbias = cst + Cfg::CB_UPT;
        {
            const int pl = L - 1 - o;
            if (pl >= p_lo && pl < p_hi) {
                const float *wf = packed + weight_offset(1 + stage + 1);
                for (int i = tid; i < PADT * COT; i += NCONS) {
                    const int co = i / PADT, j = i - co * PADT;
                    const float *wp = wf + ((size_t)co * S + j) * 2 + 1;
                    float acc0 = 0.f, acc1 = 0.f, acc2 = 0.f, acc3 = 0.f;
#pragma unroll 1
                    for (int cc = 0; cc < C; cc += 32) {
                        float wv[32];
#pragma unroll
                        for (int k = 0; k < 32; ++k) wv[k] = __ldg(wp + (size_t)(cc + k) * COT * S * 2);
#pragma unroll
                        for (int k = 0; k < 32; k += 4) {
                            acc0 = fmaf(b1s[cc + k], wv[k], acc0);
                            acc1 = fmaf(b1s[cc + k + 1], wv[k + 1], acc1);
                            acc2 = fmaf(b1s[cc + k + 2], wv[k + 2], acc2);
                            acc3 = fmaf(b1s[cc + k + 3], wv[k + 3], acc3);
                        }
                    }
                    y[((size_t)b * COT + co) * Lout + (size_t)S * L - PADT + j] = (acc0 + acc1) + (acc2 + acc3) + tbias[co];
                }
            }
        }
        const uint64_t tbdesc_t = desc_template(TN * 16, 128);
#pragma unroll 1
        for (int cg = 0; cg < Cfg::TNCG; ++cg) {
#pragma unroll 1
            for (int ch = 0; ch < C / 16; ++ch) {
#pragma unroll 1
                for (int ts = 0; ts < (S == 8 ? 2 : 1); ++ts) {
                    const uint64_t bbase = desc_at(tbdesc_t, chunk_begin() + c0 * 16);
#pragma unroll
                    for (int tp = 0; tp < (S == 8 ? 1 : 2); ++tp) {
                        const int tap = S == 8 ? ts : tp;
#pragma unroll
                        for (int pass = 0; pass < 3; ++pass) {
                            const uint32_t boff = (uint32_t)((((S == 8 ? 0 : tp * 2) + (pass == 2 ? 1 : 0)) * 2) * TN * 16);
                            const uint64_t bdesc = bbase + (uint64_t)(boff >> 4);
                            const uint32_t arow = (uint32_t)((SLACK + rb0 * 64 - tap) * 16 + 2 * ch * XPITCH);
                            const uint64_t adesc = desc_at(adesc_t, (pass == 1 ? xl_addr : xh_addr) + arow);
#pragma unroll
                            for (int r = 0; r < RPW; ++r)
                                wgmma_bf16<NCW>(D[r], adesc + (uint64_t)(r * 64), bdesc, !(ch == 0 && tap == 0 && pass == 0));
                        }
                    }
                    chunk_end();
                }
            }
            drain();
            if (cg == Cfg::TNCG - 1) pdl_trigger();
#pragma unroll
            for (int r = 0; r < RPW; ++r)
#pragma unroll
                for (int h = 0; h < 2; ++h) {
                    const int p = (rb0 + r) * 64 + frag_row(t, h), sg = o + p;
                    const bool own = (p >= p_lo && p < p_hi && sg < L);
                    const bool lo_ok = own && sg >= 1, hi_ok = own;
                    if constexpr (S == 8) {
                        const bool ok8 = c0 == 0 ? lo_ok : hi_ok;
                        float *yb = y + ((size_t)b * COT + cg * TNG) * Lout + (own ? 8 * sg - PADT + (c0 >> 5) : 0);
#pragma unroll
                        for (int c = 0; c < 4; ++c)
#pragma unroll
                            for (int e = 0; e < 2; ++e) {
                                const int co = 8 * c + 2 * q + e;
                                const float bj = tbias[cg * TNG + co];
                                if (ok8)
                                    *reinterpret_cast<float4 *>(yb + (size_t)co * Lout) =
                                        make_float4(D[r][4 * c + 2 * h + e] + bj, D[r][4 * (4 + c) + 2 * h + e] + bj,
                                                    D[r][4 * (8 + c) + 2 * h + e] + bj, D[r][4 * (12 + c) + 2 * h + e] + bj);
                            }
                    } else {
                        float *yb = y + (size_t)b * COT * Lout + (own ? 2 * sg - PADT : 0);
#pragma unroll
                        for (int k = 0; k < NCW / 8; ++k)
#pragma unroll
                            for (int e = 0; e < 2; ++e) {
                                const int col = c0 + frag_col(q, 4 * k + e), phi = col / TNG, co = col % TNG;
                                if (phi == 0 ? lo_ok : hi_ok) yb[(size_t)co * Lout + phi] = D[r][4 * k + 2 * h + e] + tbias[co];
                            }
                    }
                }
        }
    } else {
        pdl_trigger();
        const int b = item(), L = len();
#pragma unroll
        for (int r = 0; r < RPW; ++r)
#pragma unroll
            for (int h = 0; h < 2; ++h) {
                const int p = (rb0 + r) * 64 + frag_row(t, h), tp = o + p;
                if (p >= p_lo && p < p_hi && tp < L) {
                    float *yp = y + (size_t)b * C * Ls + tp;
#pragma unroll
                    for (int k = 0; k < NCW / 8; ++k)
#pragma unroll
                        for (int e = 0; e < 2; ++e) {
                            const int col = c0 + frag_col(q, 4 * k + e);
                            yp[(size_t)col * Ls] = R[r][4 * k + 2 * h + e] + pend[col];
                        }
                }
            }
    }
    if (!ok && t == 0) atomicExch(status, 3);
    if constexpr (CS > 1) cluster_sync();
    MG_TR(20);
#undef MG_TR
}

template <class Cfg>
static int launch_resblock(const float *x, float *y, const float *packed, int stage, const RunTable &batch, int *status,
                           long long *trace, cudaStream_t s) {
    static bool configured = false;
    if (!configured) {
        MG_CUDA_TRY(cudaFuncSetAttribute(resblock_tc_kernel<Cfg>, cudaFuncAttributeMaxDynamicSharedMemorySize, Cfg::SMEM_BYTES));
        configured = true;
    }
    constexpr int CS = Cfg::CS, PC = CS * Cfg::P, PVB = Cfg::PVB;
    RunTable clusters = batch;
    clusters.set_units([](int L) { return 1 + (L > PC ? (L - PC + PVB - 1) / PVB : 0); });
    const dim3 grid(CS * clusters.first[clusters.n]);
    if (trace && CS > 1) {
        cudaLaunchConfig_t cfg{};
        cfg.gridDim = grid;
        cfg.blockDim = dim3(Cfg::NT);
        cfg.dynamicSmemBytes = Cfg::SMEM_BYTES;
        cudaLaunchAttribute attr;
        attr.id = cudaLaunchAttributeClusterDimension;
        attr.val.clusterDim.x = CS;
        attr.val.clusterDim.y = attr.val.clusterDim.z = 1;
        cfg.attrs = &attr;
        cfg.numAttrs = 1;
        int n = 0;
        MG_CUDA_TRY(cudaOccupancyMaxActiveClusters(&n, resblock_tc_kernel<Cfg>, &cfg));
        const long long v = n;
        MG_CUDA_TRY(cudaMemcpy(trace + 127, &v, sizeof(v), cudaMemcpyHostToDevice));
    }
    MG_CUDA_TRY(launch_ex(resblock_tc_kernel<Cfg>, grid, dim3(Cfg::NT), Cfg::SMEM_BYTES, s, true, CS, x, y, packed, stage, clusters,
                          status, trace));
    return MG_OK;
}

template <class Cfg>
static const char *cfg_name() {
    static char buf[96];
    snprintf(buf, sizeof(buf), "resblock_tc_kernel<RbCfg<%d,%d,%d,%d,%d,%d,%d,%d,%d>>", Cfg::C, Cfg::NRB, Cfg::RPW, Cfg::NCP,
             Cfg::NSTAGE, (int)Cfg::POST, (int)Cfg::UPF, Cfg::UPT, Cfg::CS);
    return buf;
}

using Rb0 = RbCfg<256, 1, 1, 2, 4, false, false, 0, 4>;
using Rb1 = RbCfg<128, 2, 1, 1, 4, false, false, 0, 2>;
using Rb2 = RbCfg<64, 4, 1, 1, 3>;
using Rb3 = RbCfg<32, 8, 2, 1, 4>;
using Rb3Post = RbCfg<32, 8, 2, 1, 4, true>;
using Up2Rb2 = RbCfg<64, 4, 1, 1, 3, false, true>;
using Up3Rb3 = RbCfg<32, 8, 2, 1, 4, false, true>;
using Up3Rb3Post = RbCfg<32, 8, 2, 1, 4, true, true>;
using Rb0Up1 = RbCfg<256, 1, 1, 2, 4, false, false, 8>;
using Rb1Up2 = RbCfg<128, 2, 1, 1, 4, false, false, 2>;
using Rb2Up3 = RbCfg<64, 4, 1, 1, 3, false, false, 2>;

int launch_resblock_tc(const float *x, float *y, const float *packed, int stage, const RunTable &batch, int *status, cudaStream_t s,
                       long long *trace) {
    switch (stage) {
        case 0: return launch_resblock<Rb0>(x, y, packed, 0, batch, status, trace, s);
        case 1: return launch_resblock<Rb1>(x, y, packed, 1, batch, status, trace, s);
        case 2: return launch_resblock<Rb2>(x, y, packed, 2, batch, status, trace, s);
        case 3: return launch_resblock<Rb3>(x, y, packed, 3, batch, status, trace, s);
        case 4: return launch_resblock<Rb3Post>(x, y, packed, 3, batch, status, trace, s);
        case 12: return launch_resblock<Up2Rb2>(x, y, packed, 2, batch, status, trace, s);
        case 13: return launch_resblock<Up3Rb3>(x, y, packed, 3, batch, status, trace, s);
        case 14: return launch_resblock<Up3Rb3Post>(x, y, packed, 3, batch, status, trace, s);
        case 20: return launch_resblock<Rb0Up1>(x, y, packed, 0, batch, status, trace, s);
        case 21: return launch_resblock<Rb1Up2>(x, y, packed, 1, batch, status, trace, s);
        case 22: return launch_resblock<Rb2Up3>(x, y, packed, 2, batch, status, trace, s);
    }
    return set_error(MG_ERR_INVALID_ARGUMENT, "launch_resblock_tc: stage %d", stage);
}

const char *resblock_config_name(int stage, int L) {
    (void)L;
    switch (stage) {
        case 0: return cfg_name<Rb0>();
        case 1: return cfg_name<Rb1>();
        case 2: return cfg_name<Rb2>();
        case 3: return cfg_name<Rb3>();
        case 4: return cfg_name<Rb3Post>();
        case 12: return cfg_name<Up2Rb2>();
        case 13: return cfg_name<Up3Rb3>();
        case 14: return cfg_name<Up3Rb3Post>();
        case 20: return cfg_name<Rb0Up1>();
        case 21: return cfg_name<Rb1Up2>();
        case 22: return cfg_name<Rb2Up3>();
    }
    return "";
}

}
```

### melgan_multi_b200/csrc/mg_tc.cuh

```cuda
#pragma once
#include <cuda_bf16.h>
#include <stdint.h>

namespace mg {
namespace tc {

__device__ __forceinline__ uint32_t smem_u32(const void *p) { return (uint32_t)__cvta_generic_to_shared(p); }

__device__ __forceinline__ void mbar_init(uint64_t *bar, uint32_t count) {
    asm volatile("mbarrier.init.shared::cta.b64 [%0], %1;" ::"r"(smem_u32(bar)), "r"(count));
}
__device__ __forceinline__ void fence_mbar_init() { asm volatile("fence.mbarrier_init.release.cluster;" ::: "memory"); }
__device__ __forceinline__ void mbar_arrive_expect_tx(uint64_t *bar, uint32_t bytes) {
    asm volatile("mbarrier.arrive.expect_tx.shared::cta.b64 _, [%0], %1;" ::"r"(smem_u32(bar)), "r"(bytes) : "memory");
}
__device__ __forceinline__ void mbar_arrive(uint64_t *bar) {
    asm volatile("mbarrier.arrive.shared::cta.b64 _, [%0];" ::"r"(smem_u32(bar)) : "memory");
}
__device__ __forceinline__ bool mbar_try_wait(uint64_t *bar, uint32_t parity) {
    uint32_t ok;
    asm volatile(
        "{\n\t.reg .pred p;\n\t"
        "mbarrier.try_wait.parity.shared::cta.b64 p, [%1], %2;\n\t"
        "selp.b32 %0, 1, 0, p;\n\t}"
        : "=r"(ok)
        : "r"(smem_u32(bar)), "r"(parity)
        : "memory");
    return ok != 0;
}
__device__ __forceinline__ bool mbar_wait(uint64_t *bar, uint32_t parity, uint32_t max_spins = 1u << 24) {
    for (uint32_t i = 0; i < max_spins; ++i)
        if (mbar_try_wait(bar, parity)) return true;
    return false;
}

__device__ __forceinline__ uint32_t mapa(uint32_t addr, uint32_t rank) {
    uint32_t r;
    asm volatile("mapa.shared::cluster.u32 %0, %1, %2;" : "=r"(r) : "r"(addr), "r"(rank));
    return r;
}
__device__ __forceinline__ void mbar_arrive_remote(uint64_t *bar, uint32_t rank) {
    asm volatile("mbarrier.arrive.shared::cluster.b64 _, [%0];" ::"r"(mapa(smem_u32(bar), rank)) : "memory");
}
__device__ __forceinline__ void cluster_sync() {
    asm volatile("barrier.cluster.arrive.release;\n\tbarrier.cluster.wait.acquire;" ::: "memory");
}

__device__ __forceinline__ void bulk_g2s(void *smem_dst, const void *gmem_src, uint32_t bytes, uint64_t *bar) {
    asm volatile("cp.async.bulk.shared::cluster.global.mbarrier::complete_tx::bytes [%0], [%1], %2, [%3];" ::"r"(
                     smem_u32(smem_dst)),
                 "l"(gmem_src), "r"(bytes), "r"(smem_u32(bar))
                 : "memory");
}
__device__ __forceinline__ void bulk_g2s_multicast(void *smem_dst, const void *gmem_src, uint32_t bytes, uint64_t *bar,
                                                   uint16_t cta_mask) {
    asm volatile(
        "cp.async.bulk.shared::cluster.global.mbarrier::complete_tx::bytes.multicast::cluster [%0], [%1], %2, [%3], %4;" ::"r"(
            smem_u32(smem_dst)),
        "l"(gmem_src), "r"(bytes), "r"(smem_u32(bar)), "h"(cta_mask)
        : "memory");
}
__device__ __forceinline__ void bulk_s2s_cluster(uint32_t dst, uint32_t src, uint32_t bytes, uint32_t bar) {
    asm volatile("cp.async.bulk.shared::cluster.shared::cta.mbarrier::complete_tx::bytes [%0], [%1], %2, [%3];" ::"r"(dst), "r"(src),
                 "r"(bytes), "r"(bar)
                 : "memory");
}
__device__ __forceinline__ void fence_proxy_async() { asm volatile("fence.proxy.async.shared::cta;" ::: "memory"); }

__device__ __forceinline__ void named_bar_sync(int id, int count) {
    asm volatile("bar.sync %0, %1;" ::"r"(id), "r"(count) : "memory");
}

__device__ __forceinline__ void pdl_trigger() { asm volatile("griddepcontrol.launch_dependents;" ::: "memory"); }
__device__ __forceinline__ void pdl_wait() { asm volatile("griddepcontrol.wait;" ::: "memory"); }

__device__ __forceinline__ uint64_t desc_template(uint32_t lbo_bytes, uint32_t sbo_bytes) {
    return ((uint64_t)((lbo_bytes >> 4) & 0x3FFF) << 16) | ((uint64_t)((sbo_bytes >> 4) & 0x3FFF) << 32);
}
__device__ __forceinline__ uint64_t desc_at(uint64_t tmpl, uint32_t saddr) { return tmpl | (uint64_t)((saddr >> 4) & 0x3FFF); }

__device__ __forceinline__ void wgmma_fence() { asm volatile("wgmma.fence.sync.aligned;" ::: "memory"); }
__device__ __forceinline__ void wgmma_commit() { asm volatile("wgmma.commit_group.sync.aligned;" ::: "memory"); }
template <int N>
__device__ __forceinline__ void wgmma_wait() {
    asm volatile("wgmma.wait_group.sync.aligned %0;" ::"n"(N) : "memory");
}
template <int R>
__device__ __forceinline__ void acc_fence(float *d) {
#pragma unroll
    for (int i = 0; i < R; ++i) asm volatile("" : "+f"(d[i])::"memory");
}
__device__ __forceinline__ int frag_row(int t, int h) { return 16 * (t >> 5) + ((t & 31) >> 2) + 8 * h; }
__host__ __device__ constexpr int frag_col(int lane_q, int j) { return 8 * (j >> 2) + 2 * lane_q + (j & 1); }

template <int N>
__device__ __forceinline__ void wgmma_bf16(float *d, uint64_t adesc, uint64_t bdesc, uint32_t scale_d);
#define MG_D8(i) "+f"(d[i]), "+f"(d[i + 1]), "+f"(d[i + 2]), "+f"(d[i + 3]), "+f"(d[i + 4]), "+f"(d[i + 5]), "+f"(d[i + 6]), "+f"(d[i + 7])
template <> __device__ __forceinline__ void wgmma_bf16<32>(float *d, uint64_t adesc, uint64_t bdesc, uint32_t scale_d) {
    asm volatile("{\n\t.reg .pred p;\n\tsetp.ne.b32 p, %18, 0;\n\t"
                 "wgmma.mma_async.sync.aligned.m64n32k16.f32.bf16.bf16 {%0,%1,%2,%3,%4,%5,%6,%7,%8,%9,%10,%11,%12,%13,%14,%15}, %16, %17, p, 1, 1, 0, 0;\n\t}"
                 : MG_D8(0), MG_D8(8)
                 : "l"(adesc), "l"(bdesc), "r"(scale_d));
}
template <> __device__ __forceinline__ void wgmma_bf16<64>(float *d, uint64_t adesc, uint64_t bdesc, uint32_t scale_d) {
    asm volatile("{\n\t.reg .pred p;\n\tsetp.ne.b32 p, %34, 0;\n\t"
                 "wgmma.mma_async.sync.aligned.m64n64k16.f32.bf16.bf16 {%0,%1,%2,%3,%4,%5,%6,%7,%8,%9,%10,%11,%12,%13,%14,%15,%16,%17,%18,%19,%20,%21,%22,%23,%24,%25,%26,%27,%28,%29,%30,%31}, %32, %33, p, 1, 1, 0, 0;\n\t}"
                 : MG_D8(0), MG_D8(8), MG_D8(16), MG_D8(24)
                 : "l"(adesc), "l"(bdesc), "r"(scale_d));
}
template <> __device__ __forceinline__ void wgmma_bf16<128>(float *d, uint64_t adesc, uint64_t bdesc, uint32_t scale_d) {
    asm volatile("{\n\t.reg .pred p;\n\tsetp.ne.b32 p, %66, 0;\n\t"
                 "wgmma.mma_async.sync.aligned.m64n128k16.f32.bf16.bf16 {%0,%1,%2,%3,%4,%5,%6,%7,%8,%9,%10,%11,%12,%13,%14,%15,%16,%17,%18,%19,%20,%21,%22,%23,%24,%25,%26,%27,%28,%29,%30,%31,%32,%33,%34,%35,%36,%37,%38,%39,%40,%41,%42,%43,%44,%45,%46,%47,%48,%49,%50,%51,%52,%53,%54,%55,%56,%57,%58,%59,%60,%61,%62,%63}, %64, %65, p, 1, 1, 0, 0;\n\t}"
                 : MG_D8(0), MG_D8(8), MG_D8(16), MG_D8(24), MG_D8(32), MG_D8(40), MG_D8(48), MG_D8(56)
                 : "l"(adesc), "l"(bdesc), "r"(scale_d));
}
template <> __device__ __forceinline__ void wgmma_bf16<160>(float *d, uint64_t adesc, uint64_t bdesc, uint32_t scale_d) {
    asm volatile("{\n\t.reg .pred p;\n\tsetp.ne.b32 p, %82, 0;\n\t"
                 "wgmma.mma_async.sync.aligned.m64n160k16.f32.bf16.bf16 {%0,%1,%2,%3,%4,%5,%6,%7,%8,%9,%10,%11,%12,%13,%14,%15,%16,%17,%18,%19,%20,%21,%22,%23,%24,%25,%26,%27,%28,%29,%30,%31,%32,%33,%34,%35,%36,%37,%38,%39,%40,%41,%42,%43,%44,%45,%46,%47,%48,%49,%50,%51,%52,%53,%54,%55,%56,%57,%58,%59,%60,%61,%62,%63,%64,%65,%66,%67,%68,%69,%70,%71,%72,%73,%74,%75,%76,%77,%78,%79}, %80, %81, p, 1, 1, 0, 0;\n\t}"
                 : MG_D8(0), MG_D8(8), MG_D8(16), MG_D8(24), MG_D8(32), MG_D8(40), MG_D8(48), MG_D8(56), MG_D8(64), MG_D8(72)
                 : "l"(adesc), "l"(bdesc), "r"(scale_d));
}
template <> __device__ __forceinline__ void wgmma_bf16<256>(float *d, uint64_t adesc, uint64_t bdesc, uint32_t scale_d) {
    asm volatile("{\n\t.reg .pred p;\n\tsetp.ne.b32 p, %130, 0;\n\t"
                 "wgmma.mma_async.sync.aligned.m64n256k16.f32.bf16.bf16 {%0,%1,%2,%3,%4,%5,%6,%7,%8,%9,%10,%11,%12,%13,%14,%15,%16,%17,%18,%19,%20,%21,%22,%23,%24,%25,%26,%27,%28,%29,%30,%31,%32,%33,%34,%35,%36,%37,%38,%39,%40,%41,%42,%43,%44,%45,%46,%47,%48,%49,%50,%51,%52,%53,%54,%55,%56,%57,%58,%59,%60,%61,%62,%63,%64,%65,%66,%67,%68,%69,%70,%71,%72,%73,%74,%75,%76,%77,%78,%79,%80,%81,%82,%83,%84,%85,%86,%87,%88,%89,%90,%91,%92,%93,%94,%95,%96,%97,%98,%99,%100,%101,%102,%103,%104,%105,%106,%107,%108,%109,%110,%111,%112,%113,%114,%115,%116,%117,%118,%119,%120,%121,%122,%123,%124,%125,%126,%127}, %128, %129, p, 1, 1, 0, 0;\n\t}"
                 : MG_D8(0), MG_D8(8), MG_D8(16), MG_D8(24), MG_D8(32), MG_D8(40), MG_D8(48), MG_D8(56), MG_D8(64), MG_D8(72), MG_D8(80), MG_D8(88), MG_D8(96), MG_D8(104), MG_D8(112), MG_D8(120)
                 : "l"(adesc), "l"(bdesc), "r"(scale_d));
}
#undef MG_D8

__device__ __forceinline__ void split_bf16(float x, __nv_bfloat16 &hi, __nv_bfloat16 &lo) {
    hi = __float2bfloat16_rn(x);
    lo = __float2bfloat16_rn(x - __bfloat162float(hi));
}
__device__ __forceinline__ void split2_bf16(float x0, float x1, uint32_t &hi, uint32_t &lo) {
    __nv_bfloat162 h = __floats2bfloat162_rn(x0, x1);
    float2 hf = __bfloat1622float2(h);
    __nv_bfloat162 l = __floats2bfloat162_rn(x0 - hf.x, x1 - hf.y);
    hi = *reinterpret_cast<uint32_t *>(&h);
    lo = *reinterpret_cast<uint32_t *>(&l);
}

}
}
```

### melgan_multi_b200/csrc/mg_up_tc.cu

```cuda
#include "mg_common.cuh"
#include "mg_tc.cuh"

namespace mg {
using namespace tc;

template <int STAGE_>
struct UpCfg {
    static constexpr int STAGE = STAGE_;
    static constexpr int CIN = stage_cin(STAGE), COUT = stage_cout(STAGE), S = stage_stride(STAGE), PAD = stage_pad(STAGE);
    static constexpr int NG = up_ng(STAGE);
    static constexpr int NCG = COUT / NG;
    static constexpr int N = S * NG;
    static constexpr int NMW = (N > 128) ? 1 : 2;
    static constexpr int KCA = (S == 8) ? 64 : 32;
    static constexpr int ROWS = 64 * NMW;
    static constexpr int AROWS = ROWS + 8;
    static constexpr int APITCH = AROWS * 16;
    static constexpr int ASLOT = 2 * (KCA / 8) * APITCH;
    static constexpr int BSLOT = up_slot_bytes(STAGE);
    static constexpr int NSA = (CIN == KCA) ? 1 : 2, NSB = 4;
    static constexpr int NCHUNK = CIN / 16;
    static constexpr int NCONV = 128;
    static constexpr int NT = NCONV + 128 * NMW + 32;
    static constexpr int SMEM_BYTES = NSA * ASLOT + NSB * BSLOT + (2 * NSA + 2 * NSB) * 8;
    static_assert(N <= 256 && N % 16 == 0, "wgmma N");
    static_assert(SMEM_BYTES + 1024 <= 227 * 1024, "shared memory budget");
    static_assert(CIN % KCA == 0, "A slot");
};

template <class Cfg, class Row>
__device__ __forceinline__ void convt_store(const float *acc, float *__restrict__ y, const float *__restrict__ bias, int mw, int t,
                                            int cg, int Lout, Row row) {
    constexpr int S = Cfg::S, NG = Cfg::NG, COUT = Cfg::COUT, PAD = Cfg::PAD;
    static_assert(S == 8, "the stride-2 stages store through convt_stream_store");
    const int q = t & 3;
#pragma unroll
    for (int h = 0; h < 2; ++h) {
        int m = 64 * mw + frag_row(t, h);
        asm volatile("" : "+r"(m) : : "memory");
        const RunPos p = row(m);
        const int s = p.unit;
        const bool row_ok = p.item >= 0;
        const bool lo_ok = row_ok && s >= 1, hi_ok = row_ok && s <= p.len - 1;
        float *yb = y + ((size_t)(row_ok ? p.item : 0) * COUT + cg * NG) * Lout + (S * s - PAD);
#pragma unroll
        for (int c = 0; c < 4; ++c)
#pragma unroll
            for (int e = 0; e < 2; ++e) {
                const int co = 8 * c + 2 * q + e;
                const float bj = __ldg(bias + co);
                float *yp = yb + (size_t)co * Lout;
                if (lo_ok)
                    *reinterpret_cast<float4 *>(yp) =
                        make_float4(acc[4 * (0 + c) + 2 * h + e] + bj, acc[4 * (4 + c) + 2 * h + e] + bj,
                                    acc[4 * (8 + c) + 2 * h + e] + bj, acc[4 * (12 + c) + 2 * h + e] + bj);
                if (hi_ok)
                    *reinterpret_cast<float4 *>(yp + 4) =
                        make_float4(acc[4 * (16 + c) + 2 * h + e] + bj, acc[4 * (20 + c) + 2 * h + e] + bj,
                                    acc[4 * (24 + c) + 2 * h + e] + bj, acc[4 * (28 + c) + 2 * h + e] + bj);
            }
    }
}

template <class Cfg>
__global__ void __launch_bounds__(Cfg::NT, 1)
convt_tc_kernel(const float *__restrict__ x, float *__restrict__ y, const float *__restrict__ packed,
                const __grid_constant__ RunTable rows, int *__restrict__ status) {
    constexpr int CIN = Cfg::CIN, N = Cfg::N, NG = Cfg::NG;
    constexpr int ROWS = Cfg::ROWS, APITCH = Cfg::APITCH, ASLOT = Cfg::ASLOT, BSLOT = Cfg::BSLOT, KCA = Cfg::KCA;
    constexpr int NSA = Cfg::NSA, NSB = Cfg::NSB, NCHUNK = Cfg::NCHUNK, NCONV = Cfg::NCONV, NMW = Cfg::NMW;
    extern __shared__ __align__(1024) uint8_t smem[];
    uint8_t *aring = smem, *bring = smem + NSA * ASLOT;
    uint64_t *fullA = reinterpret_cast<uint64_t *>(bring + NSB * BSLOT);
    uint64_t *emptyA = fullA + NSA, *fullB = emptyA + NSA, *emptyB = fullB + NSB;

    const int tid = threadIdx.x, warp = tid >> 5, lane = tid & 31;
    const int r0 = blockIdx.x * ROWS;
    const int cg = blockIdx.y;
    const int Lin = rows.stride;

    if (tid == 0) {
        for (int s = 0; s < NSA; ++s) { mbar_init(&fullA[s], NCONV); mbar_init(&emptyA[s], NMW); }
        for (int s = 0; s < NSB; ++s) { mbar_init(&fullB[s], 1); mbar_init(&emptyB[s], NMW); }
        fence_mbar_init();
    }
    __syncthreads();

    if (warp == (NCONV + 128 * NMW) / 32) {
        if (lane == 0) {
            const uint8_t *src = reinterpret_cast<const uint8_t *>(packed) + tc_region_start() + tc_up_offset(Cfg::STAGE) +
                                 (size_t)cg * NCHUNK * BSLOT;
            int s = 0, ph = 0;
            bool ok = true;
            for (int i = 0; i < NCHUNK && ok; ++i) {
                if (!mbar_wait(&emptyB[s], ph ^ 1)) { ok = false; break; }
                mbar_arrive_expect_tx(&fullB[s], BSLOT);
                bulk_g2s(bring + s * BSLOT, src + (size_t)i * BSLOT, BSLOT, &fullB[s]);
                if (++s == NSB) { s = 0; ph ^= 1; }
            }
            if (!ok) atomicExch(status, 12);
        }
    } else if (warp >= NCONV / 32) {
        const int mw = warp / 4 - NCONV / 128, t = tid & 127;
        const uint64_t adesc_t = desc_template(APITCH, 128), bdesc_t = desc_template(N * 16, 128);
        const uint32_t aring_addr = smem_u32(aring) + mw * 64 * 16, bring_addr = smem_u32(bring);
        float acc[N / 2];
        int sa = 0, pha = 0, sb = 0, phb = 0, psb = -1, psa = -1;
        bool ok = true;
#pragma unroll 1
        for (int ca = 0; ca < CIN / KCA; ++ca) {
            ok &= mbar_wait(&fullA[sa], pha);
            const uint64_t abase = desc_at(adesc_t, aring_addr + sa * ASLOT);
#pragma unroll 1
            for (int j = 0; j < KCA / 16; ++j) {
                ok &= mbar_wait(&fullB[sb], phb);
                const uint64_t bbase = desc_at(bdesc_t, bring_addr + sb * BSLOT);
                wgmma_fence();
#pragma unroll
                for (int tap = 0; tap < 2; ++tap)
#pragma unroll
                    for (int pass = 0; pass < 3; ++pass) {
                        const int ahalf = (pass == 1), bhalf = (pass == 2);
                        const uint64_t bdesc = bbase + (uint64_t)((((tap * 2 + bhalf) * 2) * N * 16) >> 4);
                        const uint64_t adesc =
                            abase + (uint64_t)((ahalf * (KCA / 8) * APITCH + (1 - tap) * 16) >> 4) + (uint64_t)(2 * j * (APITCH >> 4));
                        wgmma_bf16<N>(acc, adesc, bdesc, (ca | j | tap | pass) != 0);
                    }
                wgmma_commit();
                wgmma_wait<1>();
                if (t == 0 && psb >= 0) {
                    mbar_arrive(&emptyB[psb]);
                    if (psa >= 0) mbar_arrive(&emptyA[psa]);
                }
                psb = sb;
                psa = (j == KCA / 16 - 1) ? sa : -1;
                if (++sb == NSB) { sb = 0; phb ^= 1; }
            }
            if (++sa == NSA) { sa = 0; pha ^= 1; }
        }
        wgmma_wait<0>();
        acc_fence<N / 2>(acc);
        if (!ok && t == 0) atomicExch(status, 13);
        pdl_trigger();
        pdl_wait();
        convt_store<Cfg>(acc, y, packed + bias_offset(1 + Cfg::STAGE) + cg * NG, mw, t, cg, Cfg::S * Lin,
                         [&](int m) { return rows.find(r0 + m); });
    } else {
        pdl_wait();
        int sa = 0, pha = 0;
        bool ok = true;
#pragma unroll 1
        for (int ca = 0; ca < CIN / KCA; ++ca) {
            if (ok && !mbar_wait(&emptyA[sa], pha ^ 1)) { ok = false; if (lane == 0) atomicExch(status, 14); }
            uint8_t *slot = aring + sa * ASLOT;
#pragma unroll 1
            for (int i = tid; i <= ROWS; i += NCONV) {
                const RunPos p = rows.find(r0 - 1 + i);
                const bool inr = p.item >= 0 && p.unit < p.len;
                const float *xp = x + ((size_t)(inr ? p.item : 0) * CIN + ca * KCA) * Lin + (inr ? p.unit : 0);
                float f[KCA];
#pragma unroll
                for (int j = 0; j < KCA; ++j) f[j] = inr ? __ldg(xp + (size_t)j * Lin) : 0.f;
#pragma unroll
                for (int kp = 0; kp < KCA / 8; ++kp) {
                    uint32_t h[4], l[4];
#pragma unroll
                    for (int e = 0; e < 4; ++e) split2_bf16(lrelu(f[8 * kp + 2 * e]), lrelu(f[8 * kp + 2 * e + 1]), h[e], l[e]);
                    *reinterpret_cast<uint4 *>(slot + kp * APITCH + i * 16) = make_uint4(h[0], h[1], h[2], h[3]);
                    *reinterpret_cast<uint4 *>(slot + (KCA / 8 + kp) * APITCH + i * 16) = make_uint4(l[0], l[1], l[2], l[3]);
                }
            }
            fence_proxy_async();
            mbar_arrive(&fullA[sa]);
            if (++sa == NSA) { sa = 0; pha ^= 1; }
        }
    }
}

static RunTable convt_rows(const RunTable &batch) {
    RunTable rows = batch;
    rows.set_units([](int Lin) { return Lin + 1; });
    return rows;
}

template <class Cfg>
static int launch_convt(const float *x, float *y, const float *packed, const RunTable &batch, int *status, cudaStream_t s) {
    static bool configured = false;
    if (!configured) {
        MG_CUDA_TRY(cudaFuncSetAttribute(convt_tc_kernel<Cfg>, cudaFuncAttributeMaxDynamicSharedMemorySize, Cfg::SMEM_BYTES));
        configured = true;
    }
    const RunTable rows = convt_rows(batch);
    dim3 grid((unsigned)((rows.first[rows.n] + Cfg::ROWS - 1) / Cfg::ROWS), Cfg::NCG);
    MG_CUDA_TRY(launch_ex(convt_tc_kernel<Cfg>, grid, dim3(Cfg::NT), Cfg::SMEM_BYTES, s, true, 1, x, y, packed, rows, status));
    return MG_OK;
}

template <class Cfg>
struct StreamCfg {
    static_assert(Cfg::S == 2 && Cfg::NCG == 1 && Cfg::NMW == 2, "streaming ConvT: stride 2, one channel group");
    static constexpr int MAXSEG = 3;
    static constexpr int AR = Cfg::ROWS + 1;
    static constexpr int XPITCH = (AR + 6 * MAXSEG + 3) & ~3;
    static constexpr int XSLOT = Cfg::KCA * XPITCH * 4;
    static constexpr int BRES = Cfg::NCHUNK * Cfg::BSLOT;
    static constexpr int NSA = 2;
    static constexpr int FIXED = BRES + NSA * Cfg::ASLOT + 256;
    static constexpr int NSX = (227 * 1024 - 1024 - FIXED) / XSLOT < 4 ? (227 * 1024 - 1024 - FIXED) / XSLOT : 4;
    static constexpr int NT = Cfg::NCONV + 128 * Cfg::NMW + 32;
    static constexpr int SMEM_BYTES = BRES + NSA * Cfg::ASLOT + NSX * XSLOT + (1 + 2 * NSA + 2 * NSX) * 8;
    static_assert(NSX >= 2 && SMEM_BYTES + 1024 <= 227 * 1024, "shared memory budget");
    static_assert(XPITCH % 4 == 0 && Cfg::KCA == 32, "staging slot: 16-byte channel rows, one channel per producer lane");
};

struct XSeg {
    int i0, n, item, u0, dst;
};
template <class SC>
__device__ __forceinline__ void tile_segments(const RunTable &rows, int r0, XSeg (&seg)[SC::MAXSEG], int &covered) {
    int i = r0 == 0 ? 1 : 0, dst = 0;
#pragma unroll
    for (int k = 0; k < SC::MAXSEG; ++k) {
        RunPos p = rows.find(r0 - 1 + i);
        if (i < SC::AR && p.item >= 0 && p.unit == p.len) p = rows.find(r0 - 1 + ++i);
        const int n = (i < SC::AR && p.item >= 0) ? min(p.len - p.unit, SC::AR - i) : 0;
        seg[k] = {i, n, p.item, p.unit, dst};
        dst += (n + 6) & ~3;
        i += n;
    }
    covered = i;
}

template <class Cfg>
__device__ __forceinline__ void convt_stream_store(const float *acc, const float (&bj)[Cfg::NG / 8][2], float *__restrict__ y, int mw,
                                                   int t, int r0, const RunTable &rows) {
    constexpr int KB = Cfg::NG / 8, COUT = Cfg::COUT;
    const int lane = t & 31, q = t & 3, g = lane >> 2;
    const int Lout = 2 * rows.stride;
#pragma unroll
    for (int h = 0; h < 2; ++h) {
        int m = 64 * mw + frag_row(t, h);
        asm volatile("" : "+r"(m) : : "memory");
        const RunPos p = rows.find(r0 + m);
        const int s = p.unit;
        const bool pair_ok = p.item >= 0 && s < p.len, lo_ok = p.item >= 0 && s >= 1;
        float *yb = y + (size_t)(p.item >= 0 ? p.item : 0) * COUT * Lout + 2 * s;
#pragma unroll
        for (int k = 0; k < KB; ++k)
#pragma unroll
            for (int e = 0; e < 2; ++e) {
                const int co = 8 * k + 2 * q + e;
                const float p0 = acc[4 * k + 2 * h + e] + bj[k][e];
                const float p1 = acc[4 * (KB + k) + 2 * h + e] + bj[k][e];
                const float nx = h == 0 ? __shfl_sync(0xffffffffu, g == 0 ? acc[4 * k + 2 + e] + bj[k][e] : p0, (lane + 4) & 31)
                                        : __shfl_down_sync(0xffffffffu, p0, 4);
                float *yp = yb + (size_t)co * Lout;
                if (h == 1 && g == 7) {
                    if (pair_ok) yp[0] = p1;
                } else if (pair_ok) {
                    *reinterpret_cast<float2 *>(yp) = make_float2(p1, nx);
                }
                if (h == 0 && g == 0 && lo_ok) yp[-1] = p0;
            }
    }
}

template <class Cfg>
__global__ void __launch_bounds__(StreamCfg<Cfg>::NT, 1)
convt_stream_tc_kernel(const float *__restrict__ x, float *__restrict__ y, const float *__restrict__ packed,
                       const __grid_constant__ RunTable rows, int ntiles, int *__restrict__ status) {
    using SC = StreamCfg<Cfg>;
    constexpr int CIN = Cfg::CIN, N = Cfg::N, NG = Cfg::NG, KCA = Cfg::KCA, NCONV = Cfg::NCONV, NMW = Cfg::NMW;
    constexpr int ROWS = Cfg::ROWS, APITCH = Cfg::APITCH, ASLOT = Cfg::ASLOT, BSLOT = Cfg::BSLOT, NCHUNK = Cfg::NCHUNK;
    constexpr int AR = SC::AR, XPITCH = SC::XPITCH, XSLOT = SC::XSLOT, NSA = SC::NSA, NSX = SC::NSX, MAXSEG = SC::MAXSEG;
    extern __shared__ __align__(1024) uint8_t smem[];
    uint8_t *bres = smem, *aring = smem + SC::BRES, *xring = aring + NSA * ASLOT;
    uint64_t *fullW = reinterpret_cast<uint64_t *>(xring + NSX * XSLOT);
    uint64_t *fullA = fullW + 1, *emptyA = fullA + NSA, *fullX = emptyA + NSA, *emptyX = fullX + NSX;

    const int tid = threadIdx.x, warp = tid >> 5, lane = tid & 31;
    const int Lin = rows.stride;

    if (tid == 0) {
        mbar_init(fullW, 1);
        for (int s = 0; s < NSA; ++s) { mbar_init(&fullA[s], NCONV); mbar_init(&emptyA[s], NMW); }
        for (int s = 0; s < NSX; ++s) { mbar_init(&fullX[s], 1); mbar_init(&emptyX[s], NCONV); }
        fence_mbar_init();
    }
    __syncthreads();

    if (warp == (NCONV + 128 * NMW) / 32) {
        if (lane == 0) {
            const uint8_t *src = reinterpret_cast<const uint8_t *>(packed) + tc_region_start() + tc_up_offset(Cfg::STAGE);
            mbar_arrive_expect_tx(fullW, SC::BRES);
            for (int i = 0; i < NCHUNK; ++i) bulk_g2s(bres + i * BSLOT, src + (size_t)i * BSLOT, BSLOT, fullW);
        }
        pdl_wait();
        int sx = 0, phx = 0;
        bool ok = true;
#pragma unroll 1
        for (int tile = blockIdx.x; tile < ntiles && ok; tile += gridDim.x) {
            const int r0 = tile * ROWS;
            XSeg seg[MAXSEG];
            int covered;
            tile_segments<SC>(rows, r0, seg, covered);
#pragma unroll 1
            for (int ca = 0; ca < CIN / KCA; ++ca) {
                ok = __shfl_sync(0xffffffffu, lane == 0 ? mbar_wait(&emptyX[sx], phx ^ 1) : false, 0);
                if (!ok) break;
                float *slot = reinterpret_cast<float *>(xring + sx * XSLOT) + lane * XPITCH;
                size_t g0[MAXSEG];
                uint32_t bytes = 0;
#pragma unroll
                for (int k = 0; k < MAXSEG; ++k) {
                    g0[k] = ((size_t)seg[k].item * CIN + ca * KCA + lane) * Lin + seg[k].u0;
                    if (seg[k].n > 0) bytes += (uint32_t)((((g0[k] + seg[k].n + 3) & ~(size_t)3) - (g0[k] & ~(size_t)3)) * 4);
                }
                const uint32_t total = __reduce_add_sync(0xffffffffu, bytes);
                if (lane == 0) mbar_arrive_expect_tx(&fullX[sx], total);
                __syncwarp();
#pragma unroll
                for (int k = 0; k < MAXSEG; ++k)
                    if (seg[k].n > 0) {
                        const size_t a = g0[k] & ~(size_t)3, e = (g0[k] + seg[k].n + 3) & ~(size_t)3;
                        bulk_g2s(slot + seg[k].dst, x + a, (uint32_t)((e - a) * 4), &fullX[sx]);
                    }
                if (++sx == NSX) { sx = 0; phx ^= 1; }
            }
        }
        if (!ok && lane == 0) atomicExch(status, 12);
    } else if (warp >= NCONV / 32) {
        const int mw = warp / 4 - NCONV / 128, t = tid & 127;
        const uint64_t adesc_t = desc_template(APITCH, 128), bdesc_t = desc_template(N * 16, 128);
        const uint32_t aring_addr = smem_u32(aring) + mw * 64 * 16, bres_addr = smem_u32(bres);
        float bj[NG / 8][2];
#pragma unroll
        for (int k = 0; k < NG / 8; ++k)
#pragma unroll
            for (int e = 0; e < 2; ++e) bj[k][e] = __ldg(packed + bias_offset(1 + Cfg::STAGE) + 8 * k + 2 * (t & 3) + e);
        float acc[N / 2];
        int sa = 0, pha = 0;
        bool ok = mbar_wait(fullW, 0);
#pragma unroll 1
        for (int tile = blockIdx.x; tile < ntiles; tile += gridDim.x) {
            int psa = -1;
#pragma unroll 1
            for (int ca = 0; ca < CIN / KCA; ++ca) {
                ok &= mbar_wait(&fullA[sa], pha);
                const uint64_t abase = desc_at(adesc_t, aring_addr + sa * ASLOT);
#pragma unroll 1
                for (int j = 0; j < KCA / 16; ++j) {
                    const uint64_t bbase = desc_at(bdesc_t, bres_addr + (ca * (KCA / 16) + j) * BSLOT);
                    wgmma_fence();
#pragma unroll
                    for (int tap = 0; tap < 2; ++tap)
#pragma unroll
                        for (int pass = 0; pass < 3; ++pass) {
                            const int ahalf = (pass == 1), bhalf = (pass == 2);
                            const uint64_t bdesc = bbase + (uint64_t)((((tap * 2 + bhalf) * 2) * N * 16) >> 4);
                            const uint64_t adesc = abase + (uint64_t)((ahalf * (KCA / 8) * APITCH + (1 - tap) * 16) >> 4) +
                                                   (uint64_t)(2 * j * (APITCH >> 4));
                            wgmma_bf16<N>(acc, adesc, bdesc, (ca | j | tap | pass) != 0);
                        }
                    wgmma_commit();
                    wgmma_wait<1>();
                    if (t == 0 && psa >= 0) mbar_arrive(&emptyA[psa]);
                    psa = (j == KCA / 16 - 1) ? sa : -1;
                }
                if (++sa == NSA) { sa = 0; pha ^= 1; }
            }
            wgmma_wait<0>();
            acc_fence<N / 2>(acc);
            if (t == 0) mbar_arrive(&emptyA[psa]);
            if (tile + (int)gridDim.x >= ntiles) pdl_trigger();
            pdl_wait();
            convt_stream_store<Cfg>(acc, bj, y, mw, t, tile * ROWS, rows);
        }
        if (!ok && t == 0) atomicExch(status, 13);
    } else {
        pdl_wait();
        int sx = 0, phx = 0, sa = 0, pha = 0;
        bool ok = true;
#pragma unroll 1
        for (int tile = blockIdx.x; tile < ntiles; tile += gridDim.x) {
            const int r0 = tile * ROWS;
            XSeg seg[MAXSEG];
            int covered;
            tile_segments<SC>(rows, r0, seg, covered);
#pragma unroll 1
            for (int ca = 0; ca < CIN / KCA; ++ca) {
                if (ok && !(mbar_wait(&fullX[sx], phx) && mbar_wait(&emptyA[sa], pha ^ 1))) {
                    ok = false;
                    atomicExch(status, 14);
                }
                const float *xs = reinterpret_cast<const float *>(xring + sx * XSLOT);
                uint8_t *slot = aring + sa * ASLOT;
#pragma unroll 1
                for (int u = tid; u < AR * (KCA / 8); u += NCONV) {
                    const int i = u % AR, kp = u / AR;
                    int off = -1;
                    uint32_t gb = 0;
#pragma unroll
                    for (int k = 0; k < MAXSEG; ++k)
                        if (i >= seg[k].i0 && i < seg[k].i0 + seg[k].n) {
                            off = seg[k].dst + i - seg[k].i0;
                            gb = ((uint32_t)seg[k].item * CIN + ca * KCA + 8 * kp) * (uint32_t)Lin + seg[k].u0;
                        }
                    float f[8];
                    if (off >= 0) {
#pragma unroll
                        for (int e = 0; e < 8; ++e) f[e] = xs[(8 * kp + e) * XPITCH + off + ((gb + e * Lin) & 3)];
                    } else {
                        const RunPos p = i >= covered ? rows.find(r0 - 1 + i) : RunPos{-1, 0, 0};
                        const bool inr = p.item >= 0 && p.unit < p.len;
                        const float *xp = x + ((size_t)(inr ? p.item : 0) * CIN + ca * KCA + 8 * kp) * Lin + (inr ? p.unit : 0);
#pragma unroll
                        for (int e = 0; e < 8; ++e) f[e] = inr ? __ldg(xp + (size_t)e * Lin) : 0.f;
                    }
                    uint32_t h[4], l[4];
#pragma unroll
                    for (int e = 0; e < 4; ++e) split2_bf16(lrelu(f[2 * e]), lrelu(f[2 * e + 1]), h[e], l[e]);
                    *reinterpret_cast<uint4 *>(slot + kp * APITCH + i * 16) = make_uint4(h[0], h[1], h[2], h[3]);
                    *reinterpret_cast<uint4 *>(slot + (KCA / 8 + kp) * APITCH + i * 16) = make_uint4(l[0], l[1], l[2], l[3]);
                }
                fence_proxy_async();
                mbar_arrive(&fullA[sa]);
                mbar_arrive(&emptyX[sx]);
                if (++sa == NSA) { sa = 0; pha ^= 1; }
                if (++sx == NSX) { sx = 0; phx ^= 1; }
            }
        }
    }
}

template <class Cfg>
static int launch_convt_stream(const float *x, float *y, const float *packed, const RunTable &batch, int *status, cudaStream_t s) {
    using SC = StreamCfg<Cfg>;
    static bool configured = false;
    if (!configured) {
        MG_CUDA_TRY(cudaFuncSetAttribute(convt_stream_tc_kernel<Cfg>, cudaFuncAttributeMaxDynamicSharedMemorySize, SC::SMEM_BYTES));
        configured = true;
    }
    if (reinterpret_cast<uintptr_t>(x) % 16 != 0)
        return set_error(MG_ERR_INVALID_ARGUMENT, "launch_convt_tc: stage %d input not 16-byte aligned", Cfg::STAGE);
    int dev = 0, sms = 0;
    MG_CUDA_TRY(cudaGetDevice(&dev));
    MG_CUDA_TRY(cudaDeviceGetAttribute(&sms, cudaDevAttrMultiProcessorCount, dev));
    const RunTable rows = convt_rows(batch);
    const int ntiles = (rows.first[rows.n] + Cfg::ROWS - 1) / Cfg::ROWS;
    const unsigned grid = (unsigned)(ntiles < sms ? ntiles : sms);
    MG_CUDA_TRY(launch_ex(convt_stream_tc_kernel<Cfg>, dim3(grid), dim3(SC::NT), SC::SMEM_BYTES, s, true, 1, x, y, packed, rows, ntiles,
                          status));
    return MG_OK;
}

template <class Cfg>
static const char *stream_cfg_name() {
    static char buf[80];
    snprintf(buf, sizeof(buf), "convt_stream_tc_kernel<StreamCfg<%d,%d,%d,%d>>", Cfg::STAGE, Cfg::ROWS, StreamCfg<Cfg>::MAXSEG,
             StreamCfg<Cfg>::NSX);
    return buf;
}

template <class Cfg>
__global__ void __launch_bounds__(Cfg::NCONV + 128 + 32, 1)
convt_resident_tc_kernel(const float *__restrict__ x, float *__restrict__ y, const float *__restrict__ packed,
                         const __grid_constant__ RunTable rows, int *__restrict__ status) {
    constexpr int CIN = Cfg::CIN, NG = Cfg::NG, N = Cfg::N, NCG = Cfg::NCG;
    constexpr int ROWS = 64, APITCH = Cfg::APITCH, BSLOT = Cfg::BSLOT, NCHUNK = Cfg::NCHUNK;
    constexpr int KPT = CIN / 8;
    constexpr int AHALF = KPT * APITCH;
    constexpr int NSB = 4, NCONV = Cfg::NCONV;
    static_assert(Cfg::S == 8 && N == 256 && Cfg::NMW == 1 && 2 * AHALF + NSB * BSLOT + 256 + ROWS * 12 <= 227 * 1024,
                  "resident ConvT shape");
    extern __shared__ __align__(1024) uint8_t smem[];
    uint8_t *abuf = smem, *bring = smem + 2 * AHALF;
    uint64_t *fullA = reinterpret_cast<uint64_t *>(bring + NSB * BSLOT);
    uint64_t *fullB = fullA + CIN / 64, *emptyB = fullB + NSB;
    RunPos *srow = reinterpret_cast<RunPos *>(emptyB + NSB);

    const int tid = threadIdx.x, warp = tid >> 5, lane = tid & 31;
    const int r0 = blockIdx.x * ROWS;
    const int Lin = rows.stride;

    if (tid == 0) {
        for (int s = 0; s < CIN / 64; ++s) mbar_init(&fullA[s], NCONV);
        for (int s = 0; s < NSB; ++s) { mbar_init(&fullB[s], 1); mbar_init(&emptyB[s], 1); }
        fence_mbar_init();
    }
    __syncthreads();

    if (warp == NCONV / 32 + 4) {
        if (lane == 0) {
            const uint8_t *src = reinterpret_cast<const uint8_t *>(packed) + tc_region_start() + tc_up_offset(Cfg::STAGE);
            int s = 0, ph = 0;
            bool ok = true;
            for (int i = 0; i < NCG * NCHUNK && ok; ++i) {
                if (!mbar_wait(&emptyB[s], ph ^ 1)) { ok = false; break; }
                mbar_arrive_expect_tx(&fullB[s], BSLOT);
                bulk_g2s(bring + s * BSLOT, src + (size_t)i * BSLOT, BSLOT, &fullB[s]);
                if (++s == NSB) { s = 0; ph ^= 1; }
            }
            if (!ok) atomicExch(status, 32);
        }
    } else if (warp >= NCONV / 32) {
        const int t = tid & 127;
        const uint64_t adesc_t = desc_template(APITCH, 128), bdesc_t = desc_template(N * 16, 128);
        const uint32_t a_addr = smem_u32(abuf), bring_addr = smem_u32(bring);
        float acc[N / 2];
        int sb = 0, phb = 0, psb = -1;
        bool ok = true;
#pragma unroll 1
        for (int cg = 0; cg < NCG; ++cg) {
#pragma unroll 1
            for (int ch = 0; ch < NCHUNK; ++ch) {
                if (cg == 0 && (ch & 3) == 0) ok &= mbar_wait(&fullA[ch >> 2], 0);
                ok &= mbar_wait(&fullB[sb], phb);
                const uint64_t bbase = desc_at(bdesc_t, bring_addr + sb * BSLOT);
                const uint64_t abase = desc_at(adesc_t, a_addr + 2 * ch * APITCH);
                wgmma_fence();
#pragma unroll
                for (int tap = 0; tap < 2; ++tap)
#pragma unroll
                    for (int pass = 0; pass < 3; ++pass) {
                        const uint64_t bdesc = bbase + (uint64_t)((((tap * 2 + (pass == 2)) * 2) * N * 16) >> 4);
                        const uint64_t adesc = abase + (uint64_t)((((pass == 1) ? AHALF : 0) + (1 - tap) * 16) >> 4);
                        wgmma_bf16<N>(acc, adesc, bdesc, (ch | tap | pass) != 0);
                    }
                wgmma_commit();
                wgmma_wait<1>();
                if (t == 0 && psb >= 0) mbar_arrive(&emptyB[psb]);
                psb = sb;
                if (++sb == NSB) { sb = 0; phb ^= 1; }
            }
            wgmma_wait<0>();
            acc_fence<N / 2>(acc);
            if (t == 0) { mbar_arrive(&emptyB[psb]); psb = -1; }
            if (cg == NCG - 1) pdl_trigger();
            if (cg == 0) pdl_wait();
            convt_store<Cfg>(acc, y, packed + bias_offset(1 + Cfg::STAGE) + cg * NG, 0, t, cg, Cfg::S * Lin,
                             [&](int m) { return ok ? srow[m] : RunPos{-1, 0, 0}; });
        }
        if (!ok && t == 0) atomicExch(status, 33);
    } else {
        pdl_wait();
#pragma unroll 1
        for (int ca = 0; ca < CIN / 64; ++ca) {
#pragma unroll 1
            for (int i = tid; i <= ROWS; i += NCONV) {
                const RunPos p = rows.find(r0 - 1 + i);
                if (ca == 0 && i > 0) srow[i - 1] = p;
                const bool inr = p.item >= 0 && p.unit < p.len;
                const float *xp = x + ((size_t)(inr ? p.item : 0) * CIN + ca * 64) * Lin + (inr ? p.unit : 0);
                float f[64];
#pragma unroll
                for (int j = 0; j < 64; ++j) f[j] = inr ? __ldg(xp + (size_t)j * Lin) : 0.f;
#pragma unroll
                for (int kp = 0; kp < 8; ++kp) {
                    uint32_t h[4], l[4];
#pragma unroll
                    for (int e = 0; e < 4; ++e) split2_bf16(lrelu(f[8 * kp + 2 * e]), lrelu(f[8 * kp + 2 * e + 1]), h[e], l[e]);
                    *reinterpret_cast<uint4 *>(abuf + (ca * 8 + kp) * APITCH + i * 16) = make_uint4(h[0], h[1], h[2], h[3]);
                    *reinterpret_cast<uint4 *>(abuf + AHALF + (ca * 8 + kp) * APITCH + i * 16) = make_uint4(l[0], l[1], l[2], l[3]);
                }
            }
            fence_proxy_async();
            mbar_arrive(&fullA[ca]);
        }
    }
}

template <class Cfg>
static int launch_convt_resident(const float *x, float *y, const float *packed, const RunTable &batch, int *status, cudaStream_t s) {
    constexpr int smem = 2 * (Cfg::CIN / 8) * Cfg::APITCH + 4 * Cfg::BSLOT + (Cfg::CIN / 64 + 2 * 4) * 8 + 64 * sizeof(RunPos);
    static bool configured = false;
    if (!configured) {
        MG_CUDA_TRY(cudaFuncSetAttribute(convt_resident_tc_kernel<Cfg>, cudaFuncAttributeMaxDynamicSharedMemorySize, smem));
        configured = true;
    }
    const RunTable rows = convt_rows(batch);
    MG_CUDA_TRY(launch_ex(convt_resident_tc_kernel<Cfg>, dim3((unsigned)((rows.first[rows.n] + 63) / 64)), dim3(Cfg::NCONV + 128 + 32),
                          smem, s, true, 1, x, y, packed, rows, status));
    return MG_OK;
}

int launch_convt_tc(const float *x, float *y, const float *packed, int stage, const RunTable &batch, int *status, cudaStream_t s) {
    switch (stage) {
        case 0: return launch_convt<UpCfg<0>>(x, y, packed, batch, status, s);
        case 1: return launch_convt_resident<UpCfg<1>>(x, y, packed, batch, status, s);
        case 2: return launch_convt_stream<UpCfg<2>>(x, y, packed, batch, status, s);
        case 3: return launch_convt_stream<UpCfg<3>>(x, y, packed, batch, status, s);
    }
    return set_error(MG_ERR_INVALID_ARGUMENT, "launch_convt_tc: stage %d", stage);
}

const char *convt_config_name(int stage) {
    switch (stage) {
        case 2: return stream_cfg_name<UpCfg<2>>();
        case 3: return stream_cfg_name<UpCfg<3>>();
    }
    return "";
}

}
```

Before: 277.1 million.

## Make resblock kernel persistent with a bulk-copy warp staging input tiles

Converts the resblock kernel from one CTA (or cluster) per tile to a persistent grid capped at resident capacity, looping over tiles and re-streaming the weight chunks for each tile. It adds a second producer warp that bulk-copies each tile's input rows into a shared IN buffer under full/empty mbarriers, so consumers read activations from shared memory instead of global __ldg. It also adds a timeline probe entry point. The intent is to cut launch and tail imbalance and to overlap input loads with compute, at the cost of more shared memory, per-tile re-init syncs, and repeated weight streaming.

```diff
diff --git a/include/melgan_b200.h b/include/melgan_b200.h
--- a/include/melgan_b200.h
+++ b/include/melgan_b200.h
@@ -54,6 +54,8 @@
 int mg_gen_resblock_post(const void *packed, const float *x, float *audio, int B, int L, void *stream);
 
 int mg_gen_resblock_trace(const void *packed, int stage, const float *x, float *y, int B, int L, long long *trace_host);
+int mg_gen_resblock_timeline(const void *packed, int stage, const float *x, float *y, int B, int L, long long *timeline_host,
+                             int max_tiles, int *tiles);
 
 int mg_gen_stage_output(const void *workspace, int which, float *out, int B, int T, void *stream);
 
diff --git a/melgan_multi_b200/csrc/mg_api.cu b/melgan_multi_b200/csrc/mg_api.cu
--- a/melgan_multi_b200/csrc/mg_api.cu
+++ b/melgan_multi_b200/csrc/mg_api.cu
@@ -318,6 +318,31 @@
     return rc;
 }
 
+int mg_gen_resblock_timeline(const void *packed, int stage, const float *x, float *y, int B, int L, long long *timeline_host,
+                             int max_tiles, int *tiles) {
+    if (!packed || !x || !y || x == y || !timeline_host || !tiles || !*resblock_config_name(stage, 0) || B < 1 || L < 1)
+        return set_error(MG_ERR_INVALID_ARGUMENT, "mg_gen_resblock_timeline: bad argument");
+    const RunTable batch = RunTable::uniform(B, L);
+    const int n = resblock_tiles(stage, batch);
+    *tiles = n;
+    if (n > max_tiles) return set_error(MG_ERR_INVALID_ARGUMENT, "mg_gen_resblock_timeline: %d tiles, room for %d", n, max_tiles);
+    int *st = nullptr;
+    long long *tl = nullptr;
+    MG_CUDA_TRY(cudaMalloc(&st, sizeof(int)));
+    MG_CUDA_TRY(cudaMalloc(&tl, 6 * sizeof(long long) * (size_t)n));
+    cudaMemset(st, 0, sizeof(int));
+    cudaMemset(tl, 0, 6 * sizeof(long long) * (size_t)n);
+    int rc = launch_resblock_tc(x, y, (const float *)packed, stage, batch, st, 0, nullptr, tl);
+    if (rc == MG_OK && cudaDeviceSynchronize() != cudaSuccess) rc = set_error(MG_ERR_CUDA, "mg_gen_resblock_timeline: kernel failed");
+    int sv = 0;
+    if (rc == MG_OK) cudaMemcpy(&sv, st, sizeof(int), cudaMemcpyDeviceToHost);
+    if (rc == MG_OK && sv) rc = set_error(MG_ERR_CUDA, "mg_gen_resblock_timeline: pipeline wait timed out (role code %d)", sv);
+    if (rc == MG_OK) cudaMemcpy(timeline_host, tl, 6 * sizeof(long long) * (size_t)n, cudaMemcpyDeviceToHost);
+    cudaFree(st);
+    cudaFree(tl);
+    return rc;
+}
+
 int mg_gen_resblock(const void *packed, int stage, const float *x, float *y, int B, int L, void *stream) {
     if (!packed || !x || !y || x == y || stage < 0 || stage > 3 || B < 1 || L < 1)
         return set_error(MG_ERR_INVALID_ARGUMENT, "mg_gen_resblock: bad argument");
diff --git a/melgan_multi_b200/csrc/mg_common.cuh b/melgan_multi_b200/csrc/mg_common.cuh
--- a/melgan_multi_b200/csrc/mg_common.cuh
+++ b/melgan_multi_b200/csrc/mg_common.cuh
@@ -190,6 +190,7 @@
 int launch_convt_tc(const float *x, float *y, const float *packed, int stage, const RunTable &batch, int *status, cudaStream_t s);
 const char *convt_config_name(int stage);
 int launch_resblock_tc(const float *x, float *y, const float *packed, int stage, const RunTable &batch, int *status, cudaStream_t s,
-                       long long *trace = nullptr);
+                       long long *trace = nullptr, long long *timeline = nullptr);
+int resblock_tiles(int stage, const RunTable &batch);
 
 }
diff --git a/melgan_multi_b200/csrc/mg_res_tc.cu b/melgan_multi_b200/csrc/mg_res_tc.cu
--- a/melgan_multi_b200/csrc/mg_res_tc.cu
+++ b/melgan_multi_b200/csrc/mg_res_tc.cu
@@ -7,7 +7,8 @@
 namespace mg {
 using namespace tc;
 
-template <int C_, int NRB_, int RPW_, int NCP_, int NSTAGE_, bool POST_ = false, bool UPF_ = false, int UPT_ = 0, int CS_ = 1>
+template <int C_, int NRB_, int RPW_, int NCP_, int NSTAGE_, bool POST_ = false, bool UPF_ = false, int UPT_ = 0, int CS_ = 1,
+          bool STAGED_ = true>
 struct RbCfg {
     static constexpr int C = C_, NRB = NRB_, RPW = RPW_, NCP = NCP_, NSTAGE = NSTAGE_, UPT = UPT_, CS = CS_;
     static constexpr bool POST = POST_;
@@ -15,7 +16,7 @@
     static constexpr int P = 64 * NRB;
     static constexpr int NWG = NRB / RPW * NCP;
     static constexpr int NCONS = 128 * NWG;
-    static constexpr int NT = NCONS + 32;
+    static constexpr int NT = NCONS + 64;
     static constexpr int NCW = C / NCP;
     static constexpr int SLACK = 16;
     static constexpr int HALO = 16 + (POST ? 3 : 0);
@@ -44,7 +45,13 @@
     static constexpr int CB_UPF = 6 * C, CB_UPT = CB_UPF + (UPF_ ? C : 0), CB_POST = CB_UPT + (UPT_ ? C / 2 : 0);
     static constexpr int NCONST = CB_POST + (POST_ ? 32 * 8 + 4 : 0);
     static_assert(CB_POST % 4 == 0 && NCONST % 2 == 0, "conv_post weights are read as float4, the mbarriers follow");
-    static constexpr int SMEM_BYTES = 2 * XBYTES + NSTAGE * CHUNK + (2 * C + NCONST) * 4 + (2 * NSTAGE + (CS > 1 ? 2 : 0) + 1) * 8;
+    static constexpr bool STAGED = STAGED_;
+    static_assert(STAGED || !UPF, "the fused ConvT reads its operand from IN");
+    static constexpr int ICH = UPF ? 2 * C : C, IROWS = UPF ? UROWS : P, IPITCH = (IROWS + 6) & ~3;
+    static constexpr int INBYTES = STAGED ? ICH * IPITCH * 4 : 0;
+    static_assert(UPF || IPITCH % 32 == 4, "IN pitch");
+    static constexpr int SMEM_BYTES =
+        2 * XBYTES + NSTAGE * CHUNK + INBYTES + (2 * C + NCONST) * 4 + (2 * NSTAGE + (CS > 1 ? 2 : 0) + 2 + 8) * 8;
     static_assert(SMEM_BYTES + 1024 <= 227 * 1024, "shared memory budget");
     static_assert(XPITCH / 16 < 16384, "LBO field");
     static_assert(NRB % RPW == 0 && C % NCP == 0 && NCW % 32 == 0, "warpgroup split");
@@ -59,37 +66,48 @@
 template <class Cfg>
 __global__ void __launch_bounds__(Cfg::NT, 1)
 resblock_tc_kernel(const float *__restrict__ x, float *__restrict__ y, const float *__restrict__ packed, int stage,
-                   const __grid_constant__ RunTable clusters, int *__restrict__ status, long long *__restrict__ trace) {
+                   const __grid_constant__ RunTable clusters, int *__restrict__ status, long long *__restrict__ trace,
+                   long long *__restrict__ timeline) {
+    const long long tl_entry = clock64();
     constexpr int C = Cfg::C, P = Cfg::P, SLACK = Cfg::SLACK, HALO = Cfg::HALO, HL = Cfg::HL;
     constexpr int XPITCH = Cfg::XPITCH, XBYTES = Cfg::XBYTES, KC = Cfg::KC, CHUNK = Cfg::CHUNK, NSTAGE = Cfg::NSTAGE;
     constexpr int NCONS = Cfg::NCONS, NCP = Cfg::NCP, NCW = Cfg::NCW, RPW = Cfg::RPW, KSL = Cfg::KSL, NA = NCW / 2;
     constexpr int CS = Cfg::CS, XCH = Cfg::XCH;
     extern __shared__ __align__(1024) uint8_t smem[];
     uint8_t *Xh = smem, *Xl = smem + XBYTES, *ring = smem + 2 * XBYTES;
-    float *pend = reinterpret_cast<float *>(ring + NSTAGE * CHUNK);
+    float *IN = reinterpret_cast<float *>(ring + NSTAGE * CHUNK);
+    float *pend = IN + Cfg::INBYTES / 4;
     float *b1s = pend + C;
     float *cst = b1s + C;
     uint64_t *full = reinterpret_cast<uint64_t *>(cst + Cfg::NCONST);
     uint64_t *empty = full + NSTAGE;
     uint64_t *hfull = empty + NSTAGE, *hfree = hfull + 1;
-    int *item_len = reinterpret_cast<int *>(empty + NSTAGE + (CS > 1 ? 2 : 0));
+    uint64_t *in_full = empty + NSTAGE + (CS > 1 ? 2 : 0), *in_empty = in_full + 1;
+    int *item_len = reinterpret_cast<int *>(in_empty + 1);
+    long long *tl_at = reinterpret_cast<long long *>(in_empty + 5);
 
     const int tid = threadIdx.x, warp = tid >> 5, lane = tid & 31;
-    const int crank = blockIdx.x % CS;
-    const RunPos cp = clusters.find(blockIdx.x / CS);
-    const int clus = cp.unit, Ls = clusters.stride;
+    const int crank = blockIdx.x % CS, g = blockIdx.x / CS, G = gridDim.x / CS, nunits = clusters.first[clusters.n];
+    const int Ls = clusters.stride;
     auto item = [&]() { return *reinterpret_cast<volatile int *>(&item_len[0]); };
     auto len = [&]() { return *reinterpret_cast<volatile int *>(&item_len[1]); };
-    const int oc = clus == 0 ? 0 : (CS * P - HALO) + (clus - 1) * Cfg::PVB - HL;
-    const int o = oc + crank * P;
-    const int p_lo = (clus == 0 || crank > 0) ? 0 : HL, p_hi = (crank < CS - 1 || oc + CS * P >= cp.len) ? P : P - HALO;
-    const bool interior = (o >= 0 && o + P <= cp.len);
+    struct Tile {
+        int item, len, o, p_lo, p_hi;
+        bool interior;
+    };
+    auto tile_at = [&](int u) {
+        const RunPos cp = clusters.find(u);
+        const int clus = cp.unit;
+        const int oc = clus == 0 ? 0 : (CS * P - HALO) + (clus - 1) * Cfg::PVB - HL;
+        const int o = oc + crank * P;
+        return Tile{cp.item, cp.len, o, (clus == 0 || crank > 0) ? 0 : HL, (crank < CS - 1 || oc + CS * P >= cp.len) ? P : P - HALO,
+                    o + P <= cp.len};
+    };
     const int l0 = 5 + 6 * stage;
     const uint8_t *tc_base = reinterpret_cast<const uint8_t *>(packed) + tc_region_start();
 
     if (tid == 0) {
-        item_len[0] = cp.item;
-        item_len[1] = cp.len;
+        tl_at[0] = tl_entry;
         for (int s = 0; s < NSTAGE; ++s) {
             mbar_init(&full[s], 1);
             mbar_init(&empty[s], Cfg::NWG * CS);
@@ -98,6 +116,8 @@
             mbar_init(hfull, 1);
             mbar_init(hfree, (crank > 0) + (crank < CS - 1));
         }
+        mbar_init(in_full, 1);
+        mbar_init(in_empty, NCONS / 32);
         fence_mbar_init();
     }
     for (int i = Cfg::UPF ? 1 << 30 : tid; i < 2 * Cfg::KP * 2 * SLACK; i += Cfg::NT) {
@@ -105,7 +125,6 @@
         const int row = r < SLACK ? r : P + r;
         *reinterpret_cast<uint4 *>((hl ? Xl : Xh) + kp * XPITCH + row * 16) = make_uint4(0, 0, 0, 0);
     }
-    for (int i = tid; i < C; i += Cfg::NT) pend[i] = 0.f;
     for (int i = tid; i < Cfg::NCONST; i += Cfg::NT) {
         float v = 0.f;
         if (i < Cfg::CB_UPF) v = __ldg(packed + bias_offset(l0) + i);
@@ -122,7 +141,7 @@
     fence_proxy_async();
     __syncthreads();
     if constexpr (CS > 1) cluster_sync();
-    const bool tr = trace && blockIdx.x == (gridDim.x > 1 ? 1u : 0u) && tid == 0;
+    bool tr = trace && blockIdx.x == (gridDim.x > 1 ? 1u : 0u) && tid == 0;
 #define MG_TR(slot) do { if (tr) trace[slot] = clock64(); } while (0)
 
     if (warp == NCONS / 32) {
@@ -137,20 +156,48 @@
                 ++j;
                 if (++s == NSTAGE) { s = 0; ph ^= 1; }
             };
-            if constexpr (Cfg::UPF) {
-                const uint8_t *src = tc_base + tc_upf_offset(stage);
-                for (int i = 0; i < Cfg::NUPCH; ++i) put(src + (size_t)i * CHUNK, CHUNK);
-            }
-            for (int conv = 0; conv < 6; ++conv) {
-                const uint8_t *src = tc_base + tc_res_offset(l0 + (conv >> 1) + 3 * (conv & 1));
-                for (int i = 0; i < Cfg::NCHUNK; ++i) put(src + (size_t)i * CHUNK, CHUNK);
-            }
-            if constexpr (Cfg::UPT != 0) {
-                const uint8_t *src = tc_base + tc_up_offset(stage + 1);
-                for (int i = 0; i < Cfg::TNSLOT; ++i) put(src + (size_t)i * Cfg::TSLOT, Cfg::TSLOT);
+#pragma unroll 1
+            for (int u = g; u < nunits && ok; u += G) {
+                if constexpr (Cfg::UPF) {
+                    const uint8_t *src = tc_base + tc_upf_offset(stage);
+                    for (int i = 0; i < Cfg::NUPCH; ++i) put(src + (size_t)i * CHUNK, CHUNK);
+                }
+                for (int conv = 0; conv < 6; ++conv) {
+                    const uint8_t *src = tc_base + tc_res_offset(l0 + (conv >> 1) + 3 * (conv & 1));
+                    for (int i = 0; i < Cfg::NCHUNK; ++i) put(src + (size_t)i * CHUNK, CHUNK);
+                }
+                if constexpr (Cfg::UPT != 0) {
+                    const uint8_t *src = tc_base + tc_up_offset(stage + 1);
+                    for (int i = 0; i < Cfg::TNSLOT; ++i) put(src + (size_t)i * Cfg::TSLOT, Cfg::TSLOT);
+                }
             }
             if (!ok) atomicExch(status, 2);
         }
+        if constexpr (CS > 1) cluster_sync();
+        return;
+    }
+    if (warp == NCONS / 32 + 1) {
+        pdl_wait();
+        bool ok = true;
+        int k = 0;
+#pragma unroll 1
+        for (int u = g; Cfg::STAGED && u < nunits && ok; u += G, ++k) {
+            ok = __shfl_sync(0xffffffffu, lane == 0 ? mbar_wait(in_empty, (k & 1) ^ 1) : false, 0);
+            if (!ok) break;
+            const Tile tl = tile_at(u);
+            const int Lx = Cfg::UPF ? Ls >> 1 : Ls, Lin = Cfg::UPF ? tl.len >> 1 : tl.len;
+            const int r0 = Cfg::UPF ? (tl.o >> 1) - 1 : tl.o;
+            const int first = max(r0, 0), n = min(r0 + Cfg::IROWS, Lin) - first;
+            uint32_t bytes = 0;
+            for (int c = lane; c < Cfg::ICH; c += 32) bytes += aligned_span_bytes(((size_t)tl.item * Cfg::ICH + c) * Lx + first, n);
+            const uint32_t total = __reduce_add_sync(0xffffffffu, bytes);
+            if (lane == 0) mbar_arrive_expect_tx(in_full, total);
+            __syncwarp();
+            if (n > 0)
+                for (int c = lane; c < Cfg::ICH; c += 32)
+                    bulk_span_g2s(IN + c * Cfg::IPITCH, x, ((size_t)tl.item * Cfg::ICH + c) * Lx + first, n, in_full);
+        }
+        if (!ok && lane == 0) atomicExch(status, 4);
         if constexpr (CS > 1) cluster_sync();
         return;
     }
@@ -191,6 +238,10 @@
         ps = -1;
     };
     auto sync_cons = [&]() { named_bar_sync(1, NCONS); };
+    auto t_o = [&]() { return *reinterpret_cast<volatile int *>(&item_len[3]); };
+    auto t_plo = [&]() { return *reinterpret_cast<volatile int *>(&item_len[4]); };
+    auto t_phi = [&]() { return *reinterpret_cast<volatile int *>(&item_len[5]); };
+    auto t_interior = [&]() { return *reinterpret_cast<volatile int *>(&item_len[6]) != 0; };
     const int nbr = tid == 0 ? crank - 1 : crank + 1;
     const bool tells = tid < 2 && nbr >= 0 && nbr < CS;
     auto x_read = [&]() {
@@ -199,7 +250,8 @@
             if (tells) mbar_arrive_remote(hfree, nbr);
     };
     auto write_x = [&](float (&A)[RPW][NA], const float *bsrc, bool keep_last) {
-        const int L = len();
+        const int L = len(), o = t_o();
+        const bool interior = t_interior();
 #pragma unroll
         for (int r = 0; r < RPW; ++r)
 #pragma unroll
@@ -288,24 +340,61 @@
 
     pdl_wait();
     MG_TR(0);
+    if (timeline && tid == 0) tl_at[1] = clock64();
+    auto unit = [&]() { return *reinterpret_cast<volatile int *>(&item_len[2]); };
+    auto last = [&]() { return unit() + gridDim.x / CS >= clusters.first[clusters.n]; };
+#pragma unroll 1
+    for (int u = blockIdx.x / CS; u < clusters.first[clusters.n]; u = unit() + gridDim.x / CS) {
+    {
+        if (timeline && tid == 0) tl_at[2] = clock64();
+        sync_cons();
+        if (tid == 0) {
+            const Tile tl = tile_at(u);
+            item_len[0] = tl.item;
+            item_len[1] = tl.len;
+            item_len[2] = u;
+            item_len[7] = (u - g) / G & 1;
+            item_len[3] = tl.o;
+            item_len[4] = tl.p_lo;
+            item_len[5] = tl.p_hi;
+            item_len[6] = tl.interior;
+        }
+        for (int c = tid; c < C; c += NCONS) pend[c] = 0.f;
+        if constexpr (Cfg::POST && !Cfg::UPF)
+            for (int i = tid; i < 2 * Cfg::KP * 2 * SLACK; i += NCONS) {
+                const int r = i % (2 * SLACK), kp = (i / (2 * SLACK)) % Cfg::KP, hl = i / (2 * SLACK * Cfg::KP);
+                const int row = r < SLACK ? r : P + r;
+                *reinterpret_cast<uint4 *>((hl ? Xl : Xh) + kp * XPITCH + row * 16) = make_uint4(0, 0, 0, 0);
+            }
+        sync_cons();
+    }
+#pragma unroll
+    for (int r = 0; r < RPW; ++r)
+#pragma unroll
+        for (int j = 0; j < NA; ++j) R[r][j] = D[r][j] = 0.f;
+    if constexpr (Cfg::STAGED) ok &= mbar_wait(in_full, item_len[7]);
     if constexpr (Cfg::UPF) {
         constexpr int UROWS = Cfg::UROWS, UPITCH = Cfg::UPITCH, SPITCH = Cfg::SPITCH, UKSL = Cfg::UKSL;
         const int b = item(), L = len();
-        const int Lin = L >> 1, Lins = Ls >> 1, s0 = (o >> 1) - 1;
+        const int o = t_o(), Lin = L >> 1, Lins = Ls >> 1, s0 = (o >> 1) - 1;
+        const int first = max(s0, 0);
 #pragma unroll 1
         for (int idx = tid; idx < UROWS * 2 * Cfg::KP; idx += NCONS) {
             const int i = idx % UROWS, kp = idx / UROWS, sp = s0 + i;
             const bool inr = (sp >= 0 && sp < Lin);
-            const float *xp = x + ((size_t)b * 2 * C + 8 * kp) * Lins + (inr ? sp : 0);
+            const uint32_t gb = ((uint32_t)b * 2 * C + 8 * kp) * (uint32_t)Lins + first;
+            const float *xs = IN + 8 * kp * Cfg::IPITCH + sp - first;
             float f[8];
 #pragma unroll
-            for (int j = 0; j < 8; ++j) f[j] = inr ? lrelu(__ldg(xp + (size_t)j * Lins)) : 0.f;
+            for (int j = 0; j < 8; ++j) f[j] = inr ? lrelu(xs[j * Cfg::IPITCH + ((gb + j * Lins) & 3)]) : 0.f;
             uint32_t h[4], l[4];
 #pragma unroll
             for (int e = 0; e < 4; ++e) split2_bf16(f[2 * e], f[2 * e + 1], h[e], l[e]);
             *reinterpret_cast<uint4 *>(Xh + kp * UPITCH + i * 16) = make_uint4(h[0], h[1], h[2], h[3]);
             *reinterpret_cast<uint4 *>(Xl + kp * UPITCH + i * 16) = make_uint4(l[0], l[1], l[2], l[3]);
         }
+        __syncwarp();
+        if (lane == 0) mbar_arrive(in_empty);
         fence_proxy_async();
         sync_cons();
         const uint64_t udesc_t = desc_template(UPITCH, 128);
@@ -366,6 +455,8 @@
         }
     } else {
         const int b = item(), L = len();
+        const int o = t_o();
+        const uint32_t gb = (uint32_t)b * C * (uint32_t)Ls + o;
 #pragma unroll
         for (int r = 0; r < RPW; ++r)
 #pragma unroll
@@ -376,12 +467,22 @@
 #pragma unroll
                 for (int k = 0; k < NCW / 8; ++k)
 #pragma unroll
-                    for (int e = 0; e < 2; ++e)
-                        R[r][4 * k + 2 * h + e] = inr ? __ldg(xp + (size_t)(c0 + frag_col(q, 4 * k + e)) * Ls) : 0.f;
-            }
+                    for (int e = 0; e < 2; ++e) {
+                        const int col = c0 + frag_col(q, 4 * k + e);
+                        if constexpr (Cfg::STAGED)
+                            R[r][4 * k + 2 * h + e] = inr ? IN[col * Cfg::IPITCH + p + ((gb + col * Ls) & 3)] : 0.f;
+                        else
+                            R[r][4 * k + 2 * h + e] = inr ? __ldg(xp + (size_t)col * Ls) : 0.f;
+                    }
+            }
+        if constexpr (Cfg::STAGED) {
+            __syncwarp();
+            if (lane == 0) mbar_arrive(in_empty);
+        }
     }
     hand_off(R, pend, false);
     MG_TR(1);
+    if (timeline && tid == 0) tl_at[3] = clock64();
 
 #pragma unroll 1
     for (int pr = 0; pr < 3; ++pr) {
@@ -401,8 +502,9 @@
     }
 
     if constexpr (Cfg::POST) {
-        pdl_trigger();
+        if (last()) pdl_trigger();
         float *Q = reinterpret_cast<float *>(Xh);
+        const int o = t_o();
         const float *wpost = cst + Cfg::CB_POST;
 #pragma unroll
         for (int r = 0; r < RPW; ++r)
@@ -436,7 +538,7 @@
                 }
             }
         sync_cons();
-        const int b = item(), L = len();
+        const int b = item(), L = len(), p_lo = t_plo(), p_hi = t_phi();
         const float bpost = cst[Cfg::CB_POST + 32 * 8];
 #pragma unroll 1
         for (int p = tid; p < P; p += NCONS) {
@@ -451,11 +553,11 @@
                 y[(size_t)b * Ls + tp] = tanhf(acc);
             }
         }
-        if (oc + P >= L)
+        if (o + P >= L)
             for (int p = L + tid; p < Ls; p += NCONS) y[(size_t)b * Ls + p] = 0.f;
     } else if constexpr (Cfg::UPT != 0) {
         constexpr int S = Cfg::UPT, TNG = Cfg::TNG, TN = Cfg::TN, PADT = S / 2, COT = C / 2;
-        const int b = item(), L = len();
+        const int b = item(), L = len(), o = t_o(), p_lo = t_plo(), p_hi = t_phi();
         const int Lout = S * Ls;
         const float *tbias = cst + Cfg::CB_UPT;
         {
@@ -509,7 +611,7 @@
                 }
             }
             drain();
-            if (cg == Cfg::TNCG - 1) pdl_trigger();
+            if (cg == Cfg::TNCG - 1 && last()) pdl_trigger();
 #pragma unroll
             for (int r = 0; r < RPW; ++r)
 #pragma unroll
@@ -544,8 +646,8 @@
                 }
         }
     } else {
-        pdl_trigger();
-        const int b = item(), L = len();
+        if (last()) pdl_trigger();
+        const int b = item(), L = len(), o = t_o(), p_lo = t_plo(), p_hi = t_phi();
 #pragma unroll
         for (int r = 0; r < RPW; ++r)
 #pragma unroll
@@ -563,42 +665,70 @@
                 }
             }
     }
+    MG_TR(20);
+    tr = false;
+    if (timeline && tid == 0) {
+        uint32_t smid;
+        asm volatile("mov.u32 %0, %%smid;" : "=r"(smid));
+        long long *rec = timeline + 6 * ((size_t)unit() * CS + crank);
+        rec[0] = smid; rec[1] = tl_at[0]; rec[2] = tl_at[1]; rec[3] = tl_at[2]; rec[4] = tl_at[3]; rec[5] = clock64();
+    }
+    }
     if (!ok && t == 0) atomicExch(status, 3);
     if constexpr (CS > 1) cluster_sync();
-    MG_TR(20);
 #undef MG_TR
+}
+
+template <class Cfg>
+static RunTable cluster_units(const RunTable &batch) {
+    constexpr int PC = Cfg::CS * Cfg::P, PVB = Cfg::PVB;
+    RunTable clusters = batch;
+    clusters.set_units([](int L) { return 1 + (L > PC ? (L - PC + PVB - 1) / PVB : 0); });
+    return clusters;
 }
 
 template <class Cfg>
 static int launch_resblock(const float *x, float *y, const float *packed, int stage, const RunTable &batch, int *status,
-                           long long *trace, cudaStream_t s) {
+                           long long *trace, long long *timeline, cudaStream_t s) {
     static bool configured = false;
     if (!configured) {
         MG_CUDA_TRY(cudaFuncSetAttribute(resblock_tc_kernel<Cfg>, cudaFuncAttributeMaxDynamicSharedMemorySize, Cfg::SMEM_BYTES));
         configured = true;
     }
-    constexpr int CS = Cfg::CS, PC = CS * Cfg::P, PVB = Cfg::PVB;
-    RunTable clusters = batch;
-    clusters.set_units([](int L) { return 1 + (L > PC ? (L - PC + PVB - 1) / PVB : 0); });
-    const dim3 grid(CS * clusters.first[clusters.n]);
+    if (reinterpret_cast<uintptr_t>(x) % 16 != 0)
+        return set_error(MG_ERR_INVALID_ARGUMENT, "launch_resblock_tc: input not 16-byte aligned");
+    constexpr int CS = Cfg::CS;
+    static int capacity = 0;
+    if (!capacity) {
+        int dev = 0, n = 0;
+        MG_CUDA_TRY(cudaGetDevice(&dev));
+        if (CS == 1) {
+            MG_CUDA_TRY(cudaDeviceGetAttribute(&n, cudaDevAttrMultiProcessorCount, dev));
+        } else {
+            cudaLaunchConfig_t cfg{};
+            cfg.gridDim = dim3(CS);
+            cfg.blockDim = dim3(Cfg::NT);
+            cfg.dynamicSmemBytes = Cfg::SMEM_BYTES;
+            cudaLaunchAttribute attr;
+            attr.id = cudaLaunchAttributeClusterDimension;
+            attr.val.clusterDim.x = CS;
+            attr.val.clusterDim.y = attr.val.clusterDim.z = 1;
+            cfg.attrs = &attr;
+            cfg.numAttrs = 1;
+            MG_CUDA_TRY(cudaOccupancyMaxActiveClusters(&n, resblock_tc_kernel<Cfg>, &cfg));
+        }
+        if (n < 1) return set_error(MG_ERR_CUDA, "launch_resblock_tc: no resident cluster of %d CTAs", CS);
+        capacity = n;
+    }
+    const RunTable clusters = cluster_units<Cfg>(batch);
+    const int units = clusters.first[clusters.n], rounds = (units + capacity - 1) / capacity;
+    const dim3 grid(CS * ((units + rounds - 1) / rounds));
     if (trace && CS > 1) {
-        cudaLaunchConfig_t cfg{};
-        cfg.gridDim = grid;
-        cfg.blockDim = dim3(Cfg::NT);
-        cfg.dynamicSmemBytes = Cfg::SMEM_BYTES;
-        cudaLaunchAttribute attr;
-        attr.id = cudaLaunchAttributeClusterDimension;
-        attr.val.clusterDim.x = CS;
-        attr.val.clusterDim.y = attr.val.clusterDim.z = 1;
-        cfg.attrs = &attr;
-        cfg.numAttrs = 1;
-        int n = 0;
-        MG_CUDA_TRY(cudaOccupancyMaxActiveClusters(&n, resblock_tc_kernel<Cfg>, &cfg));
-        const long long v = n;
+        const long long v = capacity;
         MG_CUDA_TRY(cudaMemcpy(trace + 127, &v, sizeof(v), cudaMemcpyHostToDevice));
     }
     MG_CUDA_TRY(launch_ex(resblock_tc_kernel<Cfg>, grid, dim3(Cfg::NT), Cfg::SMEM_BYTES, s, true, CS, x, y, packed, stage, clusters,
-                          status, trace));
+                          status, trace, timeline));
     return MG_OK;
 }
 
@@ -610,7 +740,7 @@
     return buf;
 }
 
-using Rb0 = RbCfg<256, 1, 1, 2, 4, false, false, 0, 4>;
+using Rb0 = RbCfg<256, 1, 1, 2, 4, false, false, 0, 4, false>;
 using Rb1 = RbCfg<128, 2, 1, 1, 4, false, false, 0, 2>;
 using Rb2 = RbCfg<64, 4, 1, 1, 3>;
 using Rb3 = RbCfg<32, 8, 2, 1, 4>;
@@ -618,44 +748,46 @@
 using Up2Rb2 = RbCfg<64, 4, 1, 1, 3, false, true>;
 using Up3Rb3 = RbCfg<32, 8, 2, 1, 4, false, true>;
 using Up3Rb3Post = RbCfg<32, 8, 2, 1, 4, true, true>;
-using Rb0Up1 = RbCfg<256, 1, 1, 2, 4, false, false, 8>;
+using Rb0Up1 = RbCfg<256, 1, 1, 2, 4, false, false, 8, 1, false>;
 using Rb1Up2 = RbCfg<128, 2, 1, 1, 4, false, false, 2>;
 using Rb2Up3 = RbCfg<64, 4, 1, 1, 3, false, false, 2>;
 
-int launch_resblock_tc(const float *x, float *y, const float *packed, int stage, const RunTable &batch, int *status, cudaStream_t s,
-                       long long *trace) {
-    switch (stage) {
-        case 0: return launch_resblock<Rb0>(x, y, packed, 0, batch, status, trace, s);
-        case 1: return launch_resblock<Rb1>(x, y, packed, 1, batch, status, trace, s);
-        case 2: return launch_resblock<Rb2>(x, y, packed, 2, batch, status, trace, s);
-        case 3: return launch_resblock<Rb3>(x, y, packed, 3, batch, status, trace, s);
-        case 4: return launch_resblock<Rb3Post>(x, y, packed, 3, batch, status, trace, s);
-        case 12: return launch_resblock<Up2Rb2>(x, y, packed, 2, batch, status, trace, s);
-        case 13: return launch_resblock<Up3Rb3>(x, y, packed, 3, batch, status, trace, s);
-        case 14: return launch_resblock<Up3Rb3Post>(x, y, packed, 3, batch, status, trace, s);
-        case 20: return launch_resblock<Rb0Up1>(x, y, packed, 0, batch, status, trace, s);
-        case 21: return launch_resblock<Rb1Up2>(x, y, packed, 1, batch, status, trace, s);
-        case 22: return launch_resblock<Rb2Up3>(x, y, packed, 2, batch, status, trace, s);
-    }
-    return set_error(MG_ERR_INVALID_ARGUMENT, "launch_resblock_tc: stage %d", stage);
-}
-
-const char *resblock_config_name(int stage, int L) {
+template <class Ret, class F>
+static Ret with_cfg(int code, Ret dflt, F f) {
+    switch (code) {
+        case 0: return f(Rb0{}, 0);
+        case 1: return f(Rb1{}, 1);
+        case 2: return f(Rb2{}, 2);
+        case 3: return f(Rb3{}, 3);
+        case 4: return f(Rb3Post{}, 3);
+        case 12: return f(Up2Rb2{}, 2);
+        case 13: return f(Up3Rb3{}, 3);
+        case 14: return f(Up3Rb3Post{}, 3);
+        case 20: return f(Rb0Up1{}, 0);
+        case 21: return f(Rb1Up2{}, 1);
+        case 22: return f(Rb2Up3{}, 2);
+    }
+    return dflt;
+}
+
+int launch_resblock_tc(const float *x, float *y, const float *packed, int code, const RunTable &batch, int *status, cudaStream_t s,
+                       long long *trace, long long *timeline) {
+    const int rc = with_cfg(code, -1, [&](auto cfg, int stage) {
+        return launch_resblock<decltype(cfg)>(x, y, packed, stage, batch, status, trace, timeline, s);
+    });
+    return rc >= 0 ? rc : set_error(MG_ERR_INVALID_ARGUMENT, "launch_resblock_tc: stage %d", code);
+}
+
+const char *resblock_config_name(int code, int L) {
     (void)L;
-    switch (stage) {
-        case 0: return cfg_name<Rb0>();
-        case 1: return cfg_name<Rb1>();
-        case 2: return cfg_name<Rb2>();
-        case 3: return cfg_name<Rb3>();
-        case 4: return cfg_name<Rb3Post>();
-        case 12: return cfg_name<Up2Rb2>();
-        case 13: return cfg_name<Up3Rb3>();
-        case 14: return cfg_name<Up3Rb3Post>();
-        case 20: return cfg_name<Rb0Up1>();
-        case 21: return cfg_name<Rb1Up2>();
-        case 22: return cfg_name<Rb2Up3>();
-    }
-    return "";
-}
-
-}
+    return with_cfg(code, "", [](auto cfg, int) { return cfg_name<decltype(cfg)>(); });
+}
+
+int resblock_tiles(int code, const RunTable &batch) {
+    return with_cfg(code, 0, [&](auto cfg, int) {
+        const RunTable c = cluster_units<decltype(cfg)>(batch);
+        return decltype(cfg)::CS * c.first[c.n];
+    });
+}
+
+}
diff --git a/melgan_multi_b200/csrc/mg_tc.cuh b/melgan_multi_b200/csrc/mg_tc.cuh
--- a/melgan_multi_b200/csrc/mg_tc.cuh
+++ b/melgan_multi_b200/csrc/mg_tc.cuh
@@ -51,6 +51,12 @@
                      smem_u32(smem_dst)),
                  "l"(gmem_src), "r"(bytes), "r"(smem_u32(bar))
                  : "memory");
+}
+__device__ __forceinline__ uint32_t aligned_span_bytes(size_t g0, int n) {
+    return n > 0 ? (uint32_t)((((g0 + n + 3) & ~(size_t)3) - (g0 & ~(size_t)3)) * 4) : 0u;
+}
+__device__ __forceinline__ void bulk_span_g2s(float *dst, const float *src, size_t g0, int n, uint64_t *bar) {
+    bulk_g2s(dst, src + (g0 & ~(size_t)3), aligned_span_bytes(g0, n), bar);
 }
 __device__ __forceinline__ void bulk_g2s_multicast(void *smem_dst, const void *gmem_src, uint32_t bytes, uint64_t *bar,
                                                    uint16_t cta_mask) {
diff --git a/melgan_multi_b200/csrc/mg_up_tc.cu b/melgan_multi_b200/csrc/mg_up_tc.cu
--- a/melgan_multi_b200/csrc/mg_up_tc.cu
+++ b/melgan_multi_b200/csrc/mg_up_tc.cu
@@ -314,17 +314,14 @@
 #pragma unroll
                 for (int k = 0; k < MAXSEG; ++k) {
                     g0[k] = ((size_t)seg[k].item * CIN + ca * KCA + lane) * Lin + seg[k].u0;
-                    if (seg[k].n > 0) bytes += (uint32_t)((((g0[k] + seg[k].n + 3) & ~(size_t)3) - (g0[k] & ~(size_t)3)) * 4);
+                    bytes += aligned_span_bytes(g0[k], seg[k].n);
                 }
                 const uint32_t total = __reduce_add_sync(0xffffffffu, bytes);
                 if (lane == 0) mbar_arrive_expect_tx(&fullX[sx], total);
                 __syncwarp();
 #pragma unroll
                 for (int k = 0; k < MAXSEG; ++k)
-                    if (seg[k].n > 0) {
-                        const size_t a = g0[k] & ~(size_t)3, e = (g0[k] + seg[k].n + 3) & ~(size_t)3;
-                        bulk_g2s(slot + seg[k].dst, x + a, (uint32_t)((e - a) * 4), &fullX[sx]);
-                    }
+                    if (seg[k].n > 0) bulk_span_g2s(slot + seg[k].dst, x, g0[k], seg[k].n, &fullX[sx]);
                 if (++sx == NSX) { sx = 0; phx ^= 1; }
             }
         }
```

New measurement: 273.3 million (median of 6 runs). About the same (-1.4%).
